# psychopa4/PFNL

Measured on AMD Instinct MI355X. Metric: HR frames/sec at 4xSR, 7-frame 128x128->512x512, higher is better.
Workload: dtype f32

## Files before the change

### include/pfnl_hip.h

```cpp
#ifndef PFNL_HIP_H
#define PFNL_HIP_H

#include <stddef.h>
#include <stdint.h>

#ifdef __cplusplus
extern "C" {
#endif

typedef struct pfnl_handle pfnl_handle;

typedef enum pfnl_status {
    PFNL_OK = 0,
    PFNL_ERR_INVALID = -1,
    PFNL_ERR_STATE = -2,
    PFNL_ERR_HIP = -3,
    PFNL_ERR_NOMEM = -4,
    PFNL_ERR_NODEVICE = -5,
    PFNL_ERR_COMM = -6,
    PFNL_ERR_RANGE = -7
} pfnl_status;

typedef struct pfnl_config {
    int32_t num_frames;
// ... 8 lines not shown
int pfnl_version(void);
int pfnl_device_count(int* count);

int pfnl_create(const pfnl_config* cfg, pfnl_handle** out);
int pfnl_destroy(pfnl_handle* h);

int pfnl_set_weight(pfnl_handle* h, const char* tf_name, const float* host,
                    const int64_t* shape, int rank);
int pfnl_missing_weights(pfnl_handle* h, int* count);
int pfnl_finalize_weights(pfnl_handle* h);

int pfnl_set_option(pfnl_handle* h, const char* key, const char* value);
int pfnl_get_option(pfnl_handle* h, const char* key, char* buf, size_t buflen);

int pfnl_forward(pfnl_handle* h, const void* in, int in_is_device, void* out, int out_is_device,
                 int B, int H, int W, void* stream);
int pfnl_forward_strip(pfnl_handle* h, const void* in, void* out, int B, int H, int W, int row0, int nrows, void* stream);
int pfnl_workspace_bytes(pfnl_handle* h, int B, int H, int W, size_t* bytes);
int pfnl_plan(pfnl_handle* h, int B, int H, int W, char* buf, size_t buflen);
int pfnl_sync(pfnl_handle* h);
int pfnl_range_reruns(pfnl_handle* h, long long* count);
int pfnl_range_flag(pfnl_handle* h, int* flagged);

int pfnl_host_alloc(size_t bytes, void** out);
int pfnl_host_free(void* p);

typedef struct pfnl_comm pfnl_comm;
#define PFNL_COMM_ID_BYTES 128
enum { PFNL_COMM_SUM = 0, PFNL_COMM_MAX = 1 };
int pfnl_comm_get_unique_id(void* id );
int pfnl_comm_init_rank(int nranks, int rank, const void* id, int device_id, pfnl_comm** out);
int pfnl_comm_init_all(int ndev, const int* devs, pfnl_comm** comms );
int pfnl_comm_destroy(pfnl_comm* c);
int pfnl_comm_rank(pfnl_comm* c, int* rank, int* nranks);
int pfnl_comm_bcast_weights(pfnl_comm* c, pfnl_handle* h, int root);
int pfnl_copy_weights(pfnl_handle* dst, pfnl_handle* src);
int pfnl_comm_bcast(pfnl_comm* c, void* dev_buf, size_t bytes, int root);
int pfnl_comm_allreduce_f64(pfnl_comm* c, double* vals, int n, int op);
int pfnl_comm_barrier(pfnl_comm* c);
int pfnl_comm_allgather(pfnl_comm* c, const float* send_dev, float* recv_dev, size_t count_per_rank, void* stream);

enum {
    PFNL_K_NL_PACK = 0, PFNL_K_NL_ATTN = 1, PFNL_K_CONV0 = 2, PFNL_K_CONV3X3 = 3,
    PFNL_K_CONV1X1 = 4, PFNL_K_MERGE1 = 5, PFNL_K_TAIL = 6, PFNL_K_COUNT = 7
};
int pfnl_profile_enable(pfnl_handle* h, int enable);
int pfnl_profile_reset(pfnl_handle* h);
int pfnl_profile_read(pfnl_handle* h, double* ms , int64_t* launches );

int pfnl_debug_tap(pfnl_handle* h, const char* name, float* host_dst, size_t count);

int pfnl_op_conv2d(const float* in, const float* kernel_host, const float* bias_host,
                   const float* addend, int add_div, const float* resid, float* out,
                   int items, int frames_per_item, int H, int W, int ksize, int cout, int act,
                   void* stream);
int pfnl_op_conv2_grouped(const float* in, const float* base, const float* kernel_host, const float* bias_host,
                          const float* resid, float* out, int clips, int frames_per_clip, int H, int W, int act,
                          void* stream);
int pfnl_op_conv3x3_accum(const float* in, const float* kernel_host, const float* bias_host, float* out, int clips,
                          int frames_per_clip, int H, int W, int cout, int act, void* stream);
int pfnl_op_conv3x3_accum_split16(const float* in, const float* kernel_host, const float* bias_host, float* out, int clips,
                                  int frames_per_clip, int H, int W, int cout, int act, void* stream);
int pfnl_op_conv1x1_stream(const float* in, const float* kernel_host, const float* bias_host, float* out,
                           int items, int frames_per_item, int HW, int act, void* stream);
int pfnl_op_conv1x1_split16(const float* in, const float* kernel_host, const float* bias_host, float* out,
                            int items, int frames_per_item, int HW, int act, void* stream);
int pfnl_op_conv3x3_bf16(const uint16_t* in, const float* kernel_host, const float* bias_host, const uint16_t* addend,
                         int add_div, const uint16_t* resid, uint16_t* out, int items, int H, int W, int act, void* stream);
int pfnl_op_conv3x3_split16(const float* in, const float* kernel_host, const float* bias_host, const float* addend, int add_div,
                            const float* resid, float* out, int items, int H, int W, int act, void* stream);
int pfnl_op_conv1_conv10_split16(const float* in, const float* k1_host, const float* b1_host, const float* k10_host,
                                 const float* b10_host, float* out1, float* base, int clips, int frames_per_clip, int H, int W,
                                 void* stream);
int pfnl_op_conv1_conv10_split16_sf0(const float* in, const float* k1_host, const float* b1_host, const float* k10_host,
                                     const float* b10_host, float* out1, float* base, int clips, int frames_per_clip, int H, int W,
                                     void* stream);
int pfnl_op_conv2_chain_sf0(const float* in, const float* kernel_host, const float* bias_host, const float* base, int add_div, const float* resid,
                            float* out, uint16_t* out_sf, int items, int H, int W, int act, void* stream);
int pfnl_op_conv2_chain_ex(const float* in, const float* kernel_host, const float* bias_host, const float* base, int add_div, const float* resid,
                           float* out, int items, int H, int W, int act, int mfma, int n_full, int split_s, int split_q, void* stream);
int pfnl_op_conv1_conv10_split16_ex(const float* in, const float* k1_host, const float* b1_host, const float* k10_host,
                                    const float* b10_host, float* out1, float* base, int clips, int frames_per_clip, int H, int W,
                                    int n_full, int split_s, int split_q, void* stream);
int pfnl_op_conv3x3_accum_split16_ex(const float* in, const float* kernel_host, const float* bias_host, float* out, int clips,
                                     int frames_per_clip, int H, int W, int cout, int act, int n_full, int split_s, int split_q, void* stream);
int pfnl_op_conv3x3_bf16_ex(const uint16_t* in, const float* kernel_host, const float* bias_host, const uint16_t* addend, int add_div,
                            const uint16_t* resid, uint16_t* out, int items, int H, int W, int act, int mfma, int n_full, int split_s,
                            int split_q, void* stream);
int pfnl_op_conv1_conv10_bf16_ex(const uint16_t* in, const float* k1_host, const float* b1_host, const float* k10_host, const float* b10_host,
                                 uint16_t* out1, uint16_t* base, int clips, int frames_per_clip, int H, int W, int mfma, int n_full, int split_s,
                                 int split_q, void* stream);
int pfnl_op_conv3x3_split16_sf(int which, const float* in, const float* kernel_host, const float* bias_host, const float* addend,
                               int add_div, const float* resid, float* out, int items, int H, int W, int act, void* stream);
int pfnl_op_conv1x1_split16_sf(const float* in, const float* kernel_host, const float* bias_host, float* out, int items,
                               int frames_per_item, int HW, int act, int in_sf, int out_sf, void* stream);
int pfnl_op_conv_small(const float* a, const float* b, int nA, int a_div, int b_mul, int nsrc, const float* kernel_host,
                       const float* bias_host, const float* resid, float* out, int items, int H, int W, int ks, int cout, int act,
                       void* stream);
int pfnl_op_conv_small_pf_block(const float* x, const float* k1_host, const float* b1_host, const float* k10_host, const float* b10_host,
                                const float* k2_host, const float* b2_host, float* inp1, float* out, int clips, int T, int H, int W,
                                void* stream);
int pfnl_op_conv1_conv10_bf16(const uint16_t* in, const float* k1_host, const float* b1_host, const float* k10_host,
                              const float* b10_host, uint16_t* out1, uint16_t* base, int clips, int frames_per_clip, int H, int W,
                              void* stream);
int pfnl_op_conv3x3_accum_bf16(const uint16_t* in, const float* kernel_host, const float* bias_host, float* out, int clips,
                               int frames_per_clip, int H, int W, int cout, int act, void* stream);
int pfnl_op_conv1x1_bf16(const uint16_t* in, const float* kernel_host, const float* bias_host, uint16_t* out, int items,
                         int frames_per_item, int HW, int act, void* stream);
int pfnl_op_conv3x3_winograd(const float* in, const float* kernel_host, const float* bias_host,
                             const float* addend, int add_div, const float* resid, float* out,
                             int items, int H, int W, int act, void* stream);
int pfnl_op_conv3x3_winograd_ws(const float* in, const float* kernel_host, const float* bias_host,
                                const float* addend, int add_div, const float* resid, float* out, int items, int H,
                                int W, int act, void* stream);
int pfnl_op_nonlocal(const float* x, const float* wg_host, const float* bg_host,
                     const float* ww_host, const float* bw_host, float* out,
                     int B, int T, int H, int W, void* stream);
int pfnl_op_nonlocal_split16(const float* x, const float* wg_host, const float* bg_host,
                     const float* ww_host, const float* bw_host, float* out,
                     int B, int T, int H, int W, void* stream);
int pfnl_op_nonlocal_f16(const float* x, const float* wg_host, const float* bg_host,
                     const float* ww_host, const float* bw_host, float* out,
                     int B, int T, int H, int W, void* stream);
int pfnl_op_nonlocal_embedded(const float* x, const float* wg_host, const float* bg_host, const float* ww_host,
                              const float* bw_host, const float* wt_host, const float* bt_host, const float* wp_host,
                              const float* bp_host, float* out, int B, int T, int H, int W, void* stream);
int pfnl_op_nonlocal_block(const float* x, const float* wg_host, const float* bg_host, const float* ww_host,
                           const float* bw_host, const float* wt_host, const float* bt_host, const float* wp_host,
                           const float* bp_host, int nltype, int sub_sample, float* out, int B, int T, int H, int W, void* stream);
int pfnl_op_conv0(const float* x, const float* kernel_host, const float* bias_host, float* out, int B, int T, int H, int W,
                  void* stream);
int pfnl_op_tail(const float* merge, const float* x, const float* kernel_host, const float* bias_host, float* out, int B,
                 int T, int H, int W, int scale, void* stream);
int pfnl_op_gather_windows(const float* frames, float* win, int F, int first, int count, int T, int H, int W, void* stream);
int pfnl_op_quantise_u8(const float* sr, uint8_t* out, size_t n, void* stream);
int pfnl_op_bicubic(const float* x, float* out, int B, int H, int W, int scale, void* stream);
int pfnl_op_blur_decimate(const float* hr, float* lr, int F, int H, int W, int scale, void* stream);
int pfnl_selftest_mfma(int device_id);

#ifdef __cplusplus
}
#endif
#endif
```

### pfnl_amd/_capi.py

```python
from __future__ import annotations

import ctypes as C
import os
from typing import Optional

_HERE = os.path.dirname(os.path.abspath(__file__))
LIB_PATH = os.environ.get("PFNL_HIP_LIB", os.path.join(_HERE, "lib", "libpfnl_hip.so"))

K_NAMES = ("nl_pack", "nl_attn", "conv0", "conv3x3", "conv1x1", "merge1", "tail")


class PFNLHipError(RuntimeError):
    """A libpfnl_hip call returned a negative status."""


class PFNLHipMissing(ImportError):
    """libpfnl_hip.so has not been built (run `python -c "import __graft_entry__ as g; g.build()"`)."""


class pfnl_config(C.Structure):
    _fields_ = [("num_frames", C.c_int32), ("scale", C.c_int32), ("mf", C.c_int32),
                ("num_block", C.c_int32), ("device_id", C.c_int32), ("reserved", C.c_int32 * 3)]


_vp, _i, _fp = C.c_void_p, C.c_int, C.POINTER(C.c_float)
SIGNATURES = {
    "pfnl_last_error": (C.c_char_p, []),
    "pfnl_version": (_i, []),
    "pfnl_device_count": (_i, [C.POINTER(_i)]),
    "pfnl_create": (_i, [C.POINTER(pfnl_config), C.POINTER(_vp)]),
    "pfnl_destroy": (_i, [_vp]),
    "pfnl_set_weight": (_i, [_vp, C.c_char_p, _vp, C.POINTER(C.c_int64), _i]),
    "pfnl_missing_weights": (_i, [_vp, C.POINTER(_i)]),
    "pfnl_finalize_weights": (_i, [_vp]),
    "pfnl_set_option": (_i, [_vp, C.c_char_p, C.c_char_p]),
    "pfnl_forward": (_i, [_vp, _vp, _i, _vp, _i, _i, _i, _i, _vp]),
    "pfnl_forward_strip": (_i, [_vp, _vp, _vp, _i, _i, _i, _i, _i, _vp]),
    "pfnl_workspace_bytes": (_i, [_vp, _i, _i, _i, C.POINTER(C.c_size_t)]),
    "pfnl_plan": (_i, [_vp, _i, _i, _i, C.c_char_p, C.c_size_t]),
    "pfnl_get_option": (_i, [_vp, C.c_char_p, C.c_char_p, C.c_size_t]),
    "pfnl_sync": (_i, [_vp]),
    "pfnl_range_reruns": (_i, [_vp, C.POINTER(C.c_longlong)]),
    "pfnl_range_flag": (_i, [_vp, C.POINTER(_i)]),
    "pfnl_host_alloc": (_i, [C.c_size_t, C.POINTER(_vp)]),
    "pfnl_host_free": (_i, [_vp]),
    "pfnl_profile_enable": (_i, [_vp, _i]),
    "pfnl_profile_reset": (_i, [_vp]),
    "pfnl_profile_read": (_i, [_vp, C.POINTER(C.c_double), C.POINTER(C.c_int64)]),
    "pfnl_debug_tap": (_i, [_vp, C.c_char_p, _vp, C.c_size_t]),
    "pfnl_op_conv2d": (_i, [_vp, _vp, _vp, _vp, _i, _vp, _vp, _i, _i, _i, _i, _i, _i, _i, _vp]),
    "pfnl_op_conv2_grouped": (_i, [_vp, _vp, _vp, _vp, _vp, _vp, _i, _i, _i, _i, _i, _vp]),
    "pfnl_op_conv3x3_accum": (_i, [_vp, _vp, _vp, _vp, _i, _i, _i, _i, _i, _i, _vp]),
    "pfnl_op_conv3x3_accum_split16": (_i, [_vp, _vp, _vp, _vp, _i, _i, _i, _i, _i, _i, _vp]),
    "pfnl_op_conv1x1_split16": (_i, [_vp, _vp, _vp, _vp, _i, _i, _i, _i, _vp]),
    "pfnl_op_conv1x1_stream": (_i, [_vp, _vp, _vp, _vp, _i, _i, _i, _i, _vp]),
    "pfnl_op_conv3x3_bf16": (_i, [_vp, _vp, _vp, _vp, _i, _vp, _vp, _i, _i, _i, _i, _vp]),
    "pfnl_op_conv1x1_bf16": (_i, [_vp, _vp, _vp, _vp, _i, _i, _i, _i, _vp]),
    "pfnl_op_conv3x3_accum_bf16": (_i, [_vp, _vp, _vp, _vp, _i, _i, _i, _i, _i, _i, _vp]),
    "pfnl_op_conv1_conv10_bf16": (_i, [_vp, _vp, _vp, _vp, _vp, _vp, _vp, _i, _i, _i, _i, _vp]),
    "pfnl_op_conv3x3_winograd": (_i, [_vp, _vp, _vp, _vp, _i, _vp, _vp, _i, _i, _i, _i, _vp]),
    "pfnl_op_conv3x3_split16": (_i, [_vp, _vp, _vp, _vp, _i, _vp, _vp, _i, _i, _i, _i, _vp]),
    "pfnl_op_conv3x3_split16_sf": (_i, [_i, _vp, _vp, _vp, _vp, _i, _vp, _vp, _i, _i, _i, _i, _vp]),
    "pfnl_op_conv_small": (_i, [_vp, _vp, _i, _i, _i, _i, _vp, _vp, _vp, _vp, _i, _i, _i, _i, _i, _i, _vp]),
    "pfnl_op_conv_small_pf_block": (_i, [_vp, _vp, _vp, _vp, _vp, _vp, _vp, _vp, _vp, _i, _i, _i, _i, _vp]),
    "pfnl_op_conv1x1_split16_sf": (_i, [_vp, _vp, _vp, _vp, _i, _i, _i, _i, _i, _i, _vp]),
    "pfnl_op_conv3x3_winograd_ws": (_i, [_vp, _vp, _vp, _vp, _i, _vp, _vp, _i, _i, _i, _i, _vp]),
    "pfnl_op_nonlocal": (_i, [_vp, _vp, _vp, _vp, _vp, _vp, _i, _i, _i, _i, _vp]),
    "pfnl_op_nonlocal_split16": (_i, [_vp, _vp, _vp, _vp, _vp, _vp, _i, _i, _i, _i, _vp]),
    "pfnl_op_nonlocal_f16": (_i, [_vp, _vp, _vp, _vp, _vp, _vp, _i, _i, _i, _i, _vp]),
    "pfnl_op_bicubic": (_i, [_vp, _vp, _i, _i, _i, _i, _vp]),
    "pfnl_op_blur_decimate": (_i, [_vp, _vp, _i, _i, _i, _i, _vp]),
    "pfnl_selftest_mfma": (_i, [_i]),
    "pfnl_op_nonlocal_embedded": (_i, [_vp, _vp, _vp, _vp, _vp, _vp, _vp, _vp, _vp, _vp, _i, _i, _i, _i, _vp]),
    "pfnl_op_conv1_conv10_split16": (_i, [_vp, _vp, _vp, _vp, _vp, _vp, _vp, _i, _i, _i, _i, _vp]),
    "pfnl_op_conv1_conv10_split16_sf0": (_i, [_vp, _vp, _vp, _vp, _vp, _vp, _vp, _i, _i, _i, _i, _vp]),
    "pfnl_op_conv2_chain_sf0": (_i, [_vp, _vp, _vp, _vp, _i, _vp, _vp, _vp, _i, _i, _i, _i, _vp]),
    "pfnl_op_conv2_chain_ex": (_i, [_vp, _vp, _vp, _vp, _i, _vp, _vp, _i, _i, _i, _i, _i, _i, _i, _i, _vp]),
    "pfnl_op_conv1_conv10_split16_ex": (_i, [_vp, _vp, _vp, _vp, _vp, _vp, _vp, _i, _i, _i, _i, _i, _i, _i, _vp]),
    "pfnl_op_conv3x3_accum_split16_ex": (_i, [_vp, _vp, _vp, _vp, _i, _i, _i, _i, _i, _i, _i, _i, _i, _vp]),
    "pfnl_op_conv3x3_bf16_ex": (_i, [_vp, _vp, _vp, _vp, _i, _vp, _vp, _i, _i, _i, _i, _i, _i, _i, _i, _vp]),
    "pfnl_op_conv1_conv10_bf16_ex": (_i, [_vp, _vp, _vp, _vp, _vp, _vp, _vp, _i, _i, _i, _i, _i, _i, _i, _i, _vp]),
    "pfnl_op_nonlocal_block": (_i, [_vp, _vp, _vp, _vp, _vp, _vp, _vp, _vp, _vp, _i, _i, _vp, _i, _i, _i, _i, _vp]),
    "pfnl_op_conv0": (_i, [_vp, _vp, _vp, _vp, _i, _i, _i, _i, _vp]),
    "pfnl_op_tail": (_i, [_vp, _vp, _vp, _vp, _vp, _i, _i, _i, _i, _i, _vp]),
    "pfnl_op_gather_windows": (_i, [_vp, _vp, _i, _i, _i, _i, _i, _i, _vp]),
    "pfnl_op_quantise_u8": (_i, [_vp, _vp, C.c_size_t, _vp]),
    "pfnl_comm_get_unique_id": (_i, [_vp]),
    "pfnl_comm_init_rank": (_i, [_i, _i, _vp, _i, C.POINTER(_vp)]),
    "pfnl_comm_init_all": (_i, [_i, C.POINTER(_i), C.POINTER(_vp)]),
    "pfnl_comm_destroy": (_i, [_vp]),
    "pfnl_comm_rank": (_i, [_vp, C.POINTER(_i), C.POINTER(_i)]),
    "pfnl_comm_bcast_weights": (_i, [_vp, _vp, _i]),
    "pfnl_copy_weights": (_i, [_vp, _vp]),
    "pfnl_comm_bcast": (_i, [_vp, _vp, C.c_size_t, _i]),
    "pfnl_comm_allreduce_f64": (_i, [_vp, C.POINTER(C.c_double), _i, _i]),
    "pfnl_comm_barrier": (_i, [_vp]),
    "pfnl_comm_allgather": (_i, [_vp, _vp, _vp, C.c_size_t, _vp]),
}
COMM_ID_BYTES = 128
COMM_SUM, COMM_MAX = 0, 1

_lib: Optional[C.CDLL] = None


def load_library(path: str = LIB_PATH) -> C.CDLL:
    global _lib
    if _lib is not None:
        return _lib
    if not os.path.exists(path):
        raise PFNLHipMissing(f"{path} not found: build it with __graft_entry__.build() "
                             f"(make -C pfnl_amd/csrc); there is no CPU fallback")
    try:
        import torch
        cand = os.path.join(os.path.dirname(torch.__file__), "lib", "librccl.so")
        if os.path.exists(cand):
            os.environ.setdefault("PFNL_RCCL_LIB", cand)
    except Exception:
        pass
    lib = C.CDLL(path, mode=C.RTLD_GLOBAL)
    for name, (res, args) in SIGNATURES.items():
        fn = getattr(lib, name)
        fn.restype = res
        fn.argtypes = args
    _lib = lib
    return lib


def check(status: int) -> None:
    if status != 0:
        msg = load_library().pfnl_last_error()
        raise PFNLHipError(f"libpfnl_hip status {status}: {msg.decode() if msg else '?'}")


def device_count() -> int:
    n = C.c_int(0)
    check(load_library().pfnl_device_count(C.byref(n)))
    return n.value
```

### pfnl_amd/csrc/capi.hip

```cpp
#include <dlfcn.h>

#include <atomic>
#include <cmath>
#include <condition_variable>
#include <cstdio>
#include <cstdlib>
#include <cstring>
#include <functional>
#include <map>
#include <memory>
#include <mutex>
#include <string>
#include <thread>
#include <vector>

#include "../../include/pfnl_hip.h"
#include "capi_internal.h"
#include "common.h"
#include "conv_bf16.h"
#include "conv_split16.h"
#include "conv_small.h"

namespace {

// ... 51 lines not shown
    }
    void release() {
        if (p) hipHostFree(p);
        p = nullptr;
        n = 0;
    }
};

struct HostPool {
    std::vector<std::thread> th;
    std::mutex m;
    std::condition_variable cv_work, cv_done;
    std::function<void(int)> fn;
    std::unique_ptr<std::atomic<int>[]> flag;
    int cap = 0, n = 0, next = 0, finished = 0, device = 0;
    bool stop = false;
    void start(int k, int dev) {
        if (!th.empty()) return;
        device = dev;
        for (int i = 0; i < k; ++i) th.emplace_back([this] { loop(); });
    }
    void loop() {
        hipSetDevice(device);
        for (;;) {
            int i;
            {
                std::unique_lock<std::mutex> lk(m);
                cv_work.wait(lk, [&] { return stop || next < n; });
                if (stop) return;
                i = next++;
            }
            fn(i);
            flag[i].store(1, std::memory_order_release);
            {
                std::lock_guard<std::mutex> lk(m);
                ++finished;
            }
            cv_done.notify_all();
        }
    }
    void run(int count, std::function<void(int)> f) {
        std::lock_guard<std::mutex> lk(m);
        if (count > cap) {
            flag.reset(new std::atomic<int>[count]);
            cap = count;
        }
        for (int i = 0; i < count; ++i) flag[i].store(0, std::memory_order_relaxed);
        fn = std::move(f);
        n = count;
        next = 0;
        finished = 0;
        cv_work.notify_all();
    }
    void wait_chunk(int i) {
        while (!flag[i].load(std::memory_order_acquire)) std::this_thread::yield();
    }
    void wait() {
        std::unique_lock<std::mutex> lk(m);
        cv_done.wait(lk, [&] { return finished >= n; });
    }
    void shutdown() {
        {
            std::lock_guard<std::mutex> lk(m);
            stop = true;
        }
        cv_work.notify_all();
        for (auto& t : th) t.join();
        th.clear();
    }
};

}

static constexpr int kSmallTiles256 = 200;
static constexpr int kMidChains256 = 136;
static int scaled_by_cus(int v256, int ncu) {
    return ncu > 0 && ncu != 256 ? std::max(1, (int)((long long)v256 * ncu / 256)) : v256;
}

struct BlockPacks {
    size_t c1_w = 0, c1_b = 0, c10_w = 0, c10_b = 0, c10_s = 0, c2a_w = 0, c2b_w = 0, c2_b = 0;
    size_t c1_u = 0, c2a_u = 0, c2b_u = 0;
    size_t bf_c1 = 0, bf_c10 = 0, bf_c2a = 0, bf_c2b = 0, bf_c1_m16 = 0, bf_c2b_m16 = 0;
    size_t s_c1 = 0, s_c2a = 0, s_c2b = 0, s_c10 = 0, s_c10f = 0, s_c2a_sf = 0, s_c2b_sf = 0, s_c2a_m16 = 0, s_c2b_m16 = 0;
    size_t sm_c1 = 0, sm_c10 = 0, sm_c2 = 0;
};

struct pfnl_handle {
    pfnl_config cfg;
    int ncu = 0;
    hipStream_t stream = nullptr;
    std::map<std::string, std::vector<int64_t>> expected;
    std::map<std::string, HostTensor> host;
    bool finalized = false;
    bool weights_external = false;
    size_t wdev_used = 0, wdev16_used = 0, wdev16s_used = 0;
    struct GraphEntry {
        int B, H, W, seen;
        hipGraph_t graph;
        hipGraphExec_t exec;
        unsigned long long alloc_gen, cfg_gen;
        unsigned long long seen_cfg_gen;
        int slot;
    };
    std::vector<GraphEntry> graphs;
    unsigned long long cfg_gen = 0;
    hipEvent_t gev = nullptr;
    int graph_mode = 0;
    bool conv2_grouped = true;
    int merge_cstride = 48;
    int conv1x1_algo = 2;
    bool bf16_fuse10 = true;
    bool bf16_m16 = true;
    bool bf16 = false;
    DevBuf wdev16;
    size_t off16_m1 = 0;
    size_t off16s_m1 = 0;
    int m1_algo = 0;
    int conv_algo = 5;
    int nl_algo = 2;
    DevBuf wdev16s;
    bool s16_m16 = true;
    size_t off16m_m1 = 0;
    unsigned* rflag_host = nullptr;
    unsigned* rflag_dev = nullptr;
    PinBuf pin_in, pin_out;
    HostPool pool;
    std::vector<hipEvent_t> d2h_ev;
    bool strict = false, strict_once = false, weights_f16_ok = true;
    long long range_reruns = 0;
    int small_mode = 0;
    bool small_c10 = true;
    DevBuf p10;
    bool sf_chain = true;
    bool sf_c10 = true;
    bool sf_mid = true;
    int sf_mid_chains = 0;
    bool sf0 = false;
    DevBuf inp0sf;
    bool split_chains = true;
    DevBuf c10part;
    bool sf_path = true;

    DevBuf wdev;
    size_t off_conv0_w = 0, off_conv0_b = 0;
    std::vector<BlockPacks> blocks;
    std::vector<size_t> off_m1_u;
    size_t off_m1_w = 0, off_m1_b = 0, off_m2_w = 0, off_m2_b = 0, off_nl_w = 0, off_nl_b = 0, off_zero = 0;

    std::map<std::string, std::vector<int64_t>> optional;
    bool nl_theta = false;
    size_t off_nl_m = 0, off_nl_c = 0;
    DevBuf Q;
    DevBuf Xs;
    int nl_type = -1;
    int nl_sub = 1;

    DevBuf nl16;
    DevBuf X, Xo, nlp, inp0, inp1, base, pb, merge, stage_in, stage_out, scratch;
    int lastB = 0, lastH = 0, lastW = 0;

    bool prof = false;
    int prof_mode = 0;
    bool prof_gate = true;
    bool chain_open = false;
    std::vector<hipEvent_t> evs;
    std::vector<int> ev_cls;
// ... 68 lines not shown
        if (h && h->prof && h->prof_gate && !h->chain_open) {
            prof_mark(h, s, -1);
            h->chain_open = true;
        }
    }
    ~ProfScope() {
        if (h && h->prof && h->prof_mode == 4) {
            h->run_cls = cls;
            ++h->run_n;
        } else if (h && h->prof && h->prof_gate) {
            prof_mark(h, s, cls);
        }
        if (ranged) roctx()->pop();
    }
};

int prof_collect(pfnl_handle* h) {
    for (size_t i = 0; i < h->evs_used; ++i) {
        const int cls = h->ev_cls[i];
        if (cls < 0 || i == 0) continue;
        if (hipEventSynchronize(h->evs[i]) != hipSuccess) return -1;
        float ms = 0.f;
        if (hipEventElapsedTime(&ms, h->evs[i - 1], h->evs[i]) != hipSuccess) return -1;
        h->prof_ms[cls] += ms;
        h->prof_n[cls] += h->ev_cnt[i];
    }
    h->evs_used = 0;
    h->chain_open = false;
    return 0;
}

int check_geometry(const pfnl_config& c) {
    if (c.num_frames != 3 && c.num_frames != 5 && c.num_frames != 7)
        return fail(PFNL_ERR_INVALID, "num_frames must be 3, 5 or 7");
    if (c.scale != 2 && c.scale != 4) return fail(PFNL_ERR_INVALID, "scale must be 2 or 4");
    if (c.mf != 64) return fail(PFNL_ERR_INVALID, "mf must be 64");
    if (c.num_block < 0 || c.num_block > 1024) return fail(PFNL_ERR_INVALID, "bad num_block");
    for (int r : c.reserved)
        if (r != 0) return fail(PFNL_ERR_INVALID, "reserved config fields must be 0");
    return 0;
}

void add_expected(pfnl_handle* h, const std::string& layer, int k, int cin, int cout) {
    h->expected["nlvsr/" + layer + "/kernel"] = {k, k, cin, cout};
    h->expected["nlvsr/" + layer + "/bias"] = {cout};
}

size_t numel(const std::vector<int64_t>& s) {
    size_t n = 1;
    for (auto d : s) n *= (size_t)d;
    return n;
}

enum Merge1Kind {
    M1_SMALL,
    M1_BF16,
    M1_SPLIT16,
    M1_SPLIT16_CUT,
    M1_WINOGRAD,
    M1_DIRECT,
};
const char* const kMerge1Names[] = {"small", "bf16", "split16", "split16_cut", "winograd", "direct"};

struct TrunkPlan {
    bool bf16 = false;
    bool strict = false;
    int nltype = 1;
    int nl_family = 0;
    bool nl_fused_pack = false;
    bool bmid = false, fuse10 = false;
    int algo = 0, conv1x1_algo = 0;
    bool sf = false;
    bool small = false, small_c10 = false;
    bool mid = false;
    bool c10_fused = false;
    bool chain = false;
    bool sf0 = false;
    bool conv2_grouped = false;
    int n_full = 0, split_s = 0, split_q = 0;
    int c1x1_launches = 0;
    int launches_per_block = 0;
    int tiles8x32 = 0, chains = 0;
    int mfma = 32;
    int merge1 = M1_DIRECT;
    int merge_stride = 48;
    size_t p10_floats = 0, inp0sf_floats = 0, c10part_floats = 0;
    const char* name = "";
};

void plan_bf16_trunk(const pfnl_handle* h, TrunkPlan& pl, int T, int grid, int mid_chains, bool fits32) {
    pl.bmid = h->sf_mid && h->bf16_fuse10 && pl.chains < mid_chains;
    pl.fuse10 = h->bf16_fuse10 && !pl.bmid;
    pl.launches_per_block = pl.fuse10 ? 3 : 4;
    pl.c1x1_launches = pl.fuse10 ? 0 : 1;
    if (pl.fuse10 && h->split_chains && fits32 && split_rule(pl.chains, T, grid, pl.n_full, pl.split_s, pl.split_q)) {
        pl.launches_per_block += 1;
        pl.c1x1_launches = 1;
    }
    pl.name = pl.bmid ? "bf16_mid4" : (pl.fuse10 ? (pl.split_s ? "bf16_3_split" : "bf16_3") : "bf16_4");
    pl.mfma = h->bf16_m16 ? 16 : 32;
    pl.merge1 = M1_BF16;
    pl.merge_stride = 64;
}

void plan_fp32_trunk(const pfnl_handle* h, TrunkPlan& pl, int B, int H, int W, int T, int grid, int mid_chains, bool fits32) {
    const int small_tiles = scaled_by_cus(kSmallTiles256, h->ncu);
    const int algo0 = h->conv_algo == 5 ? ((pl.tiles8x32 >= small_tiles && fits32) ? 4 : 3) : h->conv_algo;
    pl.algo = (pl.strict && algo0 == 4) ? 3 : algo0;
    pl.conv1x1_algo = (pl.strict && h->conv1x1_algo == 2) ? 1 : h->conv1x1_algo;
    pl.sf = pl.algo == 4 && pl.conv1x1_algo == 2 && h->sf_path;
    pl.small = !pl.strict && fits32 &&
               (h->small_mode == 1 || (h->small_mode == 0 && h->conv_algo == 5 && h->conv1x1_algo == 2 && pl.tiles8x32 < small_tiles));
    pl.small_c10 = pl.small && h->small_c10;
    if (pl.small) {
        pl.launches_per_block = pl.small_c10 ? 2 : 3;
        pl.c1x1_launches = pl.small_c10 ? 0 : 1;
        pl.name = pl.small_c10 ? "small2" : "small3";
        pl.merge1 = M1_SMALL;
        pl.merge_stride = 64;
        return;
    }
    pl.mid = pl.sf && h->sf_mid && h->conv_algo == 5 && h->sf_c10 && h->sf_chain && pl.chains < mid_chains;
    pl.c10_fused = pl.sf && h->sf_c10 && !pl.mid;
    pl.chain = pl.sf && h->sf_chain && !pl.mid;
    pl.sf0 = pl.c10_fused && pl.chain && h->sf0;
    const int wino_groups = B * ((W + 31) / 32) * ((H + 3) / 4);
    pl.conv2_grouped = pl.algo == 3 && h->conv2_grouped && wino_groups >= 224 && fits32;
    pl.launches_per_block = (pl.c10_fused ? 1 : 2) + ((pl.chain || pl.conv2_grouped) ? 1 : 2);
    pl.c1x1_launches = pl.c10_fused ? 0 : 1;
    if (pl.c10_fused && pl.chain && h->split_chains && split_rule(pl.chains, T, grid, pl.n_full, pl.split_s, pl.split_q)) {
        pl.launches_per_block += 1;
        pl.c1x1_launches = 1;
    }
    pl.mfma = (h->s16_m16 && pl.c10_fused && pl.chain && !pl.sf0 && !pl.split_s && pl.chains >= grid) ? 16 : 32;
    pl.name = pl.mid ? "mid4" : (pl.c10_fused && pl.chain) ? (pl.sf0 ? "chain2_sf0" : (pl.split_s ? "chain2_split" : "chain2"))
            : pl.algo == 4 ? (pl.launches_per_block == 3 ? "split16_3" : "split16_4")
            : pl.algo == 3 ? (pl.conv2_grouped ? "winograd_ws3" : "winograd_ws4")
            : pl.algo == 1 ? "winograd_tile4" : "direct4";
    if (pl.algo == 4 && h->m1_algo != 2 && fits32) pl.merge1 = pl.split_s ? M1_SPLIT16_CUT : M1_SPLIT16;
    else if ((pl.algo == 3 || pl.algo == 4) && wino_groups >= 224 && fits32) pl.merge1 = M1_WINOGRAD;
    pl.merge_stride = pl.merge1 == M1_DIRECT ? 48 : 64;
}

TrunkPlan trunk_plan(const pfnl_handle* h, int B, int H, int W, int Hfull) {
    TrunkPlan pl;
    const int T = h->cfg.num_frames;
    pl.bf16 = h->bf16;
    pl.strict = !h->bf16 && (h->strict || h->strict_once || !h->weights_f16_ok);
    pl.tiles8x32 = B * T * ((W + 31) / 32) * ((H + 7) / 8);
    pl.chains = pl.tiles8x32 / T;
    const int grid = persistent_grid(h->ncu);
    const int mid_chains = h->sf_mid_chains > 0 ? h->sf_mid_chains : scaled_by_cus(kMidChains256, h->ncu);
    const bool fits32 = (long long)H * W * 256 < 0x7fffffffLL;
    if (h->bf16) plan_bf16_trunk(h, pl, T, grid, mid_chains, fits32);
    else plan_fp32_trunk(h, pl, B, H, W, T, grid, mid_chains, fits32);

    const int N = (Hfull / 2) * (W / 2);
    pl.nltype = h->nl_type < 0 ? (h->nl_theta ? 0 : 1) : h->nl_type;
    pl.nl_family = (pl.nltype != 1 || h->nl_sub > 1) ? 0
                 : h->bf16 ? 2
                 : (!pl.strict && (h->nl_algo == 1 || (h->nl_algo == 2 && N >= 1024))) ? 1 : 3;
    pl.nl_fused_pack = (pl.nl_family == 1 || pl.nl_family == 2) && nl_f16_fits_one_launch(B, N);

    const size_t frame_floats = (size_t)B * T * H * W * 64;
    pl.p10_floats = pl.small_c10 ? frame_floats : 0;
    pl.inp0sf_floats = pl.sf0 ? frame_floats : 0;
    pl.c10part_floats = pl.split_s ? (size_t)(pl.chains - pl.n_full) * pl.split_s * 8 * 32 * 64 : 0;
    return pl;
}

struct Fwd {
    pfnl_handle* h;
    const TrunkPlan& pl;
    hipStream_t s;
    int B, T, F, H, W;
    const float* wd;
    const uint16_t* w16;
    const uint16_t* w16s;
};

template <class P>
void set_split_chains(P& q, const TrunkPlan& pl, float* partial) {
    q.n_full = pl.n_full;
    q.split_s = pl.split_s;
    q.split_q = pl.split_q;
    q.partial = pl.split_s ? partial : nullptr;
}

template <class P>
P split_finalize_params(const Fwd& f) {
    P q{};
    q.H = f.H;
    q.W = f.W;
    q.items = f.F;
    q.add_div = f.T;
    set_split_chains(q, f.pl, f.h->c10part.p);
    return q;
}

ConvParams direct_params(const Fwd& f, const float* in, const float* wpack, const float* bias, float* out, int cout, int frames, int act) {
    ConvParams p{};
    p.in = in;
    p.wpack = wpack;
    p.bias = bias;
    p.out = out;
    p.H = f.H;
    p.W = f.W;
    p.in_cstride = 64;
    p.out_cstride = cout;
    p.cout = cout;
    p.chunks_per_frame = 64 / CONV_CK;
    p.frames_per_item = frames;
    p.nchunks = frames * p.chunks_per_frame;
    p.add_div = 1;
    p.act = act;
    return p;
}
// ... 77 lines not shown
            q.x_bias = wd + k.c10_b;
            q.x_out = ab;
            set_split_chains(q, pl, h->c10part.p);
        }
        if (pl.mfma == 16) q.wpack16 = f.w16 + k.bf_c1_m16;
        HIPCHK(launch_conv3x3_bf16(q, s));
    }
    if (pl.fuse10 && pl.split_s) {
        ProfScope ps(h, s, PFNL_K_CONV1X1);
        ConvBf16Params q = split_finalize_params<ConvBf16Params>(f);
        q.x_bias = wd + k.c10_b;
        q.x_out = ab;
        HIPCHK(launch_c10_finalize_bf16(q, s));
    }
    if (!pl.fuse10) {
        ProfScope ps(h, s, PFNL_K_CONV1X1);
        HIPCHK(launch_conv1x1_bf16(a1, f.w16 + k.bf_c10, wd + k.c10_b, ab, f.B, f.T, f.H * f.W, 1, s));
    }
    {
        ProfScope ps(h, s, PFNL_K_CONV3X3);
        ConvBf16Params q{ab, f.w16 + k.bf_c2a, wd + h->off_zero, nullptr, nullptr, ap, f.H, f.W, f.B, 1, 0};
        HIPCHK(launch_conv3x3_bf16(q, s));
    }
    {
        ProfScope ps(h, s, PFNL_K_CONV3X3);
        ConvBf16Params q{a1, f.w16 + k.bf_c2b, wd + k.c2_b, ap, a0, a0, f.H, f.W, f.F, f.T, 1};
        q.flat = pl.bmid ? 1 : 0;
        set_split_chains(q, pl, nullptr);
        if (pl.mfma == 16) q.wpack16 = f.w16 + k.bf_c2b_m16;
        HIPCHK(launch_conv3x3_bf16(q, s));
    }
    return 0;
}

int block_small(const Fwd& f, const BlockPacks& k) {
    pfnl_handle* const h = f.h;
    const hipStream_t s = f.s;
    const float* const wd = f.wd;
    const int H = f.H, W = f.W, F = f.F, T = f.T;
    {
        ProfScope ps(h, s, PFNL_K_CONV3X3);
        ConvSmallParams q{nullptr, h->inp0.p, 0, 1, 1, 1, f.w16s + k.sm_c1, wd + k.c1_b, nullptr, h->inp1.p, H, W, F, 1, 3};
        if (f.pl.small_c10) {
            q.x_wpack = f.w16s + k.sm_c10;
            q.x_out = h->p10.p;
            q.x_T = T;
        }
        HIPCHK(launch_conv_small(q, s));
    }
    if (!f.pl.small_c10) {
        ProfScope ps(h, s, PFNL_K_CONV1X1);
        ConvSmallParams q{nullptr, h->inp1.p, 0, 1, T, T, f.w16s + k.sm_c10, wd + k.c10_b, nullptr, h->base.p, H, W, f.B, 1, 1};
        HIPCHK(launch_conv_small(q, s));
    }
    {
        ProfScope ps(h, s, PFNL_K_CONV3X3);
        ConvSmallParams q{f.pl.small_c10 ? h->p10.p : h->base.p, h->inp1.p, 1, T, 1, 2, f.w16s + k.sm_c2, wd + k.c2_b, h->inp0.p, h->inp0.p, H, W, F, 1, 3};
        if (f.pl.small_c10) {
            q.a_nsum = T;
            q.a_bias = wd + k.c10_b;
        }
        HIPCHK(launch_conv_small(q, s));
    }
    return 0;
}

int block_fp32(const Fwd& f, const BlockPacks& k, bool first, bool last) {
    pfnl_handle* const h = f.h;
    const TrunkPlan& pl = f.pl;
    const hipStream_t s = f.s;
    const float* const wd = f.wd;
    const int H = f.H, W = f.W, F = f.F, T = f.T, B = f.B, algo = pl.algo;
    const bool sf = pl.sf;
    const bool in_sf0 = pl.sf0 && !first, out_sf0 = pl.sf0 && !last;
    if (pl.c10_fused) {
        {
            ProfScope ps(h, s, PFNL_K_CONV3X3);
            ConvSplitParams q{in_sf0 ? h->inp0sf.p : h->inp0.p, f.w16s + k.s_c1, wd + k.c1_b, nullptr, nullptr, h->inp1.p, H, W, F, T, 1};
            q.in_sf = in_sf0 ? 1 : 0;
            q.wpack2 = f.w16s + k.s_c10f;
            q.bias2 = wd + k.c10_b;
            q.out2 = h->base.p;
            set_split_chains(q, pl, h->c10part.p);
            HIPCHK(launch_conv3x3_c1c10(q, s));
        }
        if (pl.split_s) {
            ProfScope ps(h, s, PFNL_K_CONV1X1);
            ConvSplitParams q = split_finalize_params<ConvSplitParams>(f);
            q.act = 1;
            q.out2 = h->base.p;
            HIPCHK(launch_c10_finalize(q, s));
        }
    } else {
        {
            ProfScope ps(h, s, PFNL_K_CONV3X3);
            if (algo == 4) {
                ConvSplitParams q{h->inp0.p, f.w16s + k.s_c1, wd + k.c1_b, nullptr, nullptr, h->inp1.p, H, W, F, 1, 1};
                q.out_sf = sf ? 1 : 0;
                HIPCHK(launch_conv3x3_split16(q, s));
            } else if (algo == 1 || algo == 3) {
                WinoParams wp{h->inp0.p, wd + k.c1_u, wd + k.c1_b, nullptr, nullptr, h->inp1.p, H, W, 1, 1, F};
                HIPCHK(algo == 3 ? launch_conv_wino_ws(wp, s) : launch_conv_wino(wp, s));
            } else {
                HIPCHK(launch_conv_mfma(direct_params(f, h->inp0.p, wd + k.c1_w, wd + k.c1_b, h->inp1.p, 64, 1, 1), 3, F, s));
            }
        }
        {
            ProfScope ps(h, s, PFNL_K_CONV1X1);
            if (pl.conv1x1_algo == 2)
                HIPCHK(launch_conv1x1_split16(h->inp1.p, f.w16s + k.s_c10, wd + k.c10_b, h->base.p, B, T, H * W, 1, s, sf, sf));
            else if (pl.conv1x1_algo == 1)
                HIPCHK(launch_conv1x1_stream(h->inp1.p, wd + k.c10_s, wd + k.c10_b, h->base.p, B, T, H * W, 1, s));
            else
                HIPCHK(launch_conv_mfma(direct_params(f, h->inp1.p, wd + k.c10_w, wd + k.c10_b, h->base.p, 64, T, 1), 1, B, s));
        }
    }
    if (pl.conv2_grouped) {
        ProfScope ps(h, s, PFNL_K_CONV3X3);
        WinoParams wp{h->inp1.p, wd + k.c2b_u, wd + k.c2_b, nullptr, h->inp0.p, h->inp0.p, H, W, T, 1, F};
        wp.in2 = h->base.p;
        wp.upack2 = wd + k.c2a_u;
        HIPCHK(launch_conv_wino_ws(wp, s));
        return 0;
    }
    if (pl.chain) {
        ProfScope ps(h, s, PFNL_K_CONV3X3);
        ConvSplitParams q{h->inp1.p, f.w16s + k.s_c2b_sf, wd + k.c2_b, nullptr, h->inp0.p, h->inp0.p, H, W, F, T, 1};
        q.in2 = h->base.p;
        q.wpack2 = f.w16s + k.s_c2a_sf;
        q.out2 = out_sf0 ? h->inp0sf.p : nullptr;
        set_split_chains(q, pl, nullptr);
        if (pl.mfma == 16) {
            q.wpack_m16 = f.w16s + k.s_c2b_m16;
            q.wpack2_m16 = f.w16s + k.s_c2a_m16;
        }
        HIPCHK(launch_conv3x3_sf_chain(q, s));
        return 0;
    }
    {
        ProfScope ps(h, s, PFNL_K_CONV3X3);
        if (algo == 4) {
            ConvSplitParams q{h->base.p, f.w16s + (sf ? k.s_c2a_sf : k.s_c2a), wd + h->off_zero, nullptr, nullptr, h->pb.p, H, W, B, 1, 0};
            HIPCHK(sf ? launch_conv3x3_sf(q, s) : launch_conv3x3_split16(q, s));
        } else if (algo == 1 || algo == 3) {
            WinoParams wp{h->base.p, wd + k.c2a_u, wd + h->off_zero, nullptr, nullptr, h->pb.p, H, W, 1, 0, B};
            HIPCHK(algo == 3 ? launch_conv_wino_ws(wp, s) : launch_conv_wino(wp, s));
        } else {
            HIPCHK(launch_conv_mfma(direct_params(f, h->base.p, wd + k.c2a_w, wd + h->off_zero, h->pb.p, 64, 1, 0), 3, B, s));
        }
    }
    {
        ProfScope ps(h, s, PFNL_K_CONV3X3);
        if (algo == 4) {
            ConvSplitParams q{h->inp1.p, f.w16s + (sf ? k.s_c2b_sf : k.s_c2b), wd + k.c2_b, h->pb.p, h->inp0.p, h->inp0.p, H, W, F, T, 1};
            q.flat = pl.mid ? 1 : 0;
            HIPCHK(sf ? launch_conv3x3_sf(q, s) : launch_conv3x3_split16(q, s));
        } else if (algo == 1 || algo == 3) {
            WinoParams wp{h->inp1.p, wd + k.c2b_u, wd + k.c2_b, h->pb.p, h->inp0.p, h->inp0.p, H, W, T, 1, F};
            HIPCHK(algo == 3 ? launch_conv_wino_ws(wp, s) : launch_conv_wino(wp, s));
        } else {
            ConvParams p = direct_params(f, h->inp1.p, wd + k.c2b_w, wd + k.c2_b, h->inp0.p, 64, 1, 1);
            p.addend = h->pb.p;
            p.add_div = T;
            p.resid = h->inp0.p;
            HIPCHK(launch_conv_mfma(p, 3, F, s));
        }
// ... 392 lines not shown
    h->blocks.assign(nb, BlockPacks{});
    for (int i = 0; i < nb; ++i) {
        const std::string s = std::to_string(i);
        BlockPacks& k = h->blocks[i];
        k.c1_w = put_pack(W("conv1_" + s), 3, 64, 0, 64, 64);
        k.c1_b = put_bias(Bv("conv1_" + s));
        k.c10_w = put_pack(W("conv10_" + s), 1, 64 * T, 0, 64 * T, 64);
        k.c10_b = put_bias(Bv("conv10_" + s));
        k.c10_s = reserve(pfnl::conv1x1_pack_floats(T));
        pfnl::conv1x1_pack_weights(W("conv10_" + s).data(), T, &blob[k.c10_s]);
        k.c2a_w = put_pack(W("conv2_" + s), 3, 128, 0, 64, 64);
        k.c2b_w = put_pack(W("conv2_" + s), 3, 128, 64, 64, 64);
        k.c2_b = put_bias(Bv("conv2_" + s));
        k.c1_u = put_wino(W("conv1_" + s), 64, 0);
        k.c2a_u = put_wino(W("conv2_" + s), 128, 0);
        k.c2b_u = put_wino(W("conv2_" + s), 128, 64);
    }
    h->off_m1_w = put_pack(W("convmerge1"), 3, 64 * T, 0, 64 * T, 48);
    h->off_m1_b = put_bias(Bv("convmerge1"));
    h->off_m1_u.assign(T, 0);
    for (int f = 0; f < T; ++f) {
        h->off_m1_u[f] = reserve(pfnl::wino_pack_floats());
        pfnl::wino_pack_weights(W("convmerge1").data(), 64 * T, 64 * f, &blob[h->off_m1_u[f]], 48);
    }
    {
        const auto& k = W("convmerge2");
        h->off_m2_w = reserve(k.size());
        std::memcpy(&blob[h->off_m2_w], k.data(), k.size() * sizeof(float));
        h->off_m2_b = put_bias(Bv("convmerge2"));
    }
    {
        h->off_nl_w = reserve((size_t)CP * CP);
        h->off_nl_b = reserve(CP);
        pfnl_nl_fold_gw(W("nlblock_0/g/g").data(), Bv("nlblock_0/g/g").data(), W("nlblock_0/w/w").data(), Bv("nlblock_0/w/w").data(), C, CP,
                        &blob[h->off_nl_w], &blob[h->off_nl_b]);
    }
    {
        int have = 0;
        for (auto& kv : h->optional) have += (int)h->host.count(kv.first);
        if (have != 0 && have != (int)h->optional.size())
            return fail(PFNL_ERR_STATE, "nlblock_0 theta/phi: all four tensors (two kernels, two biases) or none");
        h->nl_theta = have != 0;
        if (h->nl_theta) {
            h->off_nl_m = reserve((size_t)CP * CP);
            h->off_nl_c = reserve(CP);
            pfnl_nl_fold_theta_phi(W("nlblock_0/theta/theta").data(), Bv("nlblock_0/theta/theta").data(), W("nlblock_0/phi/phi").data(),
                                   Bv("nlblock_0/phi/phi").data(), C, CP, &blob[h->off_nl_m], &blob[h->off_nl_c]);
        }
    }
    {
        std::vector<uint16_t> b16;
        auto reserve16 = [&](size_t n) {
            size_t off = (b16.size() + 127) / 128 * 128;
            b16.resize(off + n, 0);
            return off;
        };
        for (int i = 0; i < nb; ++i) {
            const std::string s = std::to_string(i);
            BlockPacks& k = h->blocks[i];
            k.bf_c1 = reserve16(pfnl::conv3x3_bf16_pack_halfs());
            pfnl::conv3x3_bf16_pack_weights(W("conv1_" + s).data(), 64, 0, &b16[k.bf_c1]);
            k.bf_c10 = reserve16(pfnl::conv1x1_bf16_pack_halfs(T));
            pfnl::conv1x1_bf16_pack_weights(W("conv10_" + s).data(), T, &b16[k.bf_c10]);
            k.bf_c2a = reserve16(pfnl::conv3x3_bf16_pack_halfs());
            pfnl::conv3x3_bf16_pack_weights(W("conv2_" + s).data(), 128, 0, &b16[k.bf_c2a]);
            k.bf_c2b = reserve16(pfnl::conv3x3_bf16_pack_halfs());
            pfnl::conv3x3_bf16_pack_weights(W("conv2_" + s).data(), 128, 64, &b16[k.bf_c2b]);
            k.bf_c1_m16 = reserve16(pfnl::conv3x3_bf16_pack_halfs());
            pfnl::conv3x3_bf16_pack_weights16(W("conv1_" + s).data(), 64, 0, &b16[k.bf_c1_m16]);
            k.bf_c2b_m16 = reserve16(pfnl::conv3x3_bf16_pack_halfs());
            pfnl::conv3x3_bf16_pack_weights16(W("conv2_" + s).data(), 128, 64, &b16[k.bf_c2b_m16]);
        }
        h->off16_m1 = reserve16((size_t)T * pfnl::conv3x3_bf16_pack_halfs());
        for (int f = 0; f < T; ++f)
            pfnl::conv3x3_bf16_pack_weights(W("convmerge1").data(), 64 * T, 64 * f, &b16[h->off16_m1 + (size_t)f * pfnl::conv3x3_bf16_pack_halfs()], 48);
        b16.resize((b16.size() + 1) / 2 * 2 + 2, 0);
        h->wdev16_used = b16.size() / 2;
        if (h->wdev16.ensure(b16.size() / 2)) return fail(PFNL_ERR_NOMEM, "weight allocation failed");
        HIPCHK(hipMemcpy(h->wdev16.p, b16.data(), b16.size() * sizeof(uint16_t), hipMemcpyHostToDevice));
    }
    {
        std::vector<uint16_t> b16;
        const size_t n3 = pfnl::conv3x3_split16_pack_halfs(), n1 = pfnl::conv1x1_split16_pack_halfs(T);
        const size_t blk = 7 * n3 + n1 + pfnl::conv1x1_c10_pack_halfs(T);
        h->off16s_m1 = (size_t)nb * blk;
        const size_t m3 = pfnl::conv_small_pack_halfs(3, 1), m10 = pfnl::conv_small_pack_halfs(1, T);
        const size_t small_base = (size_t)nb * blk + (size_t)T * n3;
        h->off16m_m1 = small_base + (size_t)nb * (3 * m3 + m10);
        b16.resize(h->off16m_m1 + (size_t)T * m3 + 2, 0);
        pfnl::conv_small_pack_weights(W("convmerge1").data(), 3, T, 48, &b16[h->off16m_m1]);
        for (int f = 0; f < T; ++f)
            pfnl::conv3x3_split16_pack_weights(W("convmerge1").data(), 64 * T, 64 * f, &b16[h->off16s_m1 + (size_t)f * n3], 48);
        for (int i = 0; i < nb; ++i) {
            const std::string s = std::to_string(i);
            BlockPacks& k = h->blocks[i];
            k.s_c1 = (size_t)i * blk;
            k.s_c2a = k.s_c1 + n3;
            k.s_c2b = k.s_c1 + 2 * n3;
            k.s_c10 = k.s_c1 + 3 * n3;
            k.s_c2a_sf = k.s_c10 + n1;
            k.s_c2b_sf = k.s_c2a_sf + n3;
            k.s_c10f = k.s_c2b_sf + n3;
            k.s_c2a_m16 = k.s_c10f + pfnl::conv1x1_c10_pack_halfs(T);
            k.s_c2b_m16 = k.s_c2a_m16 + n3;
            pfnl::conv3x3_split16_pack_weights16(W("conv2_" + s).data(), 128, 0, &b16[k.s_c2a_m16]);
            pfnl::conv3x3_split16_pack_weights16(W("conv2_" + s).data(), 128, 64, &b16[k.s_c2b_m16]);
            pfnl::conv1x1_c10_pack_weights(W("conv10_" + s).data(), T, &b16[k.s_c10f]);
            pfnl::conv3x3_split16_pack_weights(W("conv2_" + s).data(), 128, 0, &b16[k.s_c2a_sf], 64, true);
            pfnl::conv3x3_split16_pack_weights(W("conv2_" + s).data(), 128, 64, &b16[k.s_c2b_sf], 64, true);
            k.sm_c1 = small_base + (size_t)i * (3 * m3 + m10);
            k.sm_c2 = k.sm_c1 + m3;
            k.sm_c10 = k.sm_c1 + 3 * m3;
            pfnl::conv_small_pack_weights(W("conv1_" + s).data(), 3, 1, 64, &b16[k.sm_c1]);
            pfnl::conv_small_pack_weights(W("conv2_" + s).data(), 3, 2, 64, &b16[k.sm_c2]);
            pfnl::conv_small_pack_weights(W("conv10_" + s).data(), 1, T, 64, &b16[k.sm_c10]);
            pfnl::conv1x1_split16_pack_weights(W("conv10_" + s).data(), T, &b16[k.s_c10]);
            pfnl::conv3x3_split16_pack_weights(W("conv1_" + s).data(), 64, 0, &b16[k.s_c1]);
            pfnl::conv3x3_split16_pack_weights(W("conv2_" + s).data(), 128, 0, &b16[k.s_c2a]);
            pfnl::conv3x3_split16_pack_weights(W("conv2_" + s).data(), 128, 64, &b16[k.s_c2b]);
        }
        h->wdev16s_used = b16.size() / 2;
        if (h->wdev16s.ensure(b16.size() / 2)) return fail(PFNL_ERR_NOMEM, "weight allocation failed");
        HIPCHK(hipMemcpy(h->wdev16s.p, b16.data(), b16.size() / 2 * 2 * sizeof(uint16_t), hipMemcpyHostToDevice));
    }
    {
        float wmax = 0.f;
        for (const auto& kv : h->host)
            for (float v : kv.second.data) wmax = std::fmax(wmax, std::fabs(v));
        h->weights_f16_ok = wmax < 65504.0f;
    }
    h->wdev_used = blob.size();
    if (h->wdev.ensure(blob.size())) return fail(PFNL_ERR_NOMEM, "weight allocation failed");
    HIPCHK(hipMemcpy(h->wdev.p, blob.data(), blob.size() * sizeof(float), hipMemcpyHostToDevice));
    h->finalized = true;
    ++h->cfg_gen;
    return 0;
}

int pfnl_workspace_bytes(pfnl_handle* h, int B, int H, int W, size_t* bytes) {
    if (!h || !bytes) return fail(PFNL_ERR_INVALID, "NULL argument");
    if (B <= 0 || H <= 0 || W <= 0 || (H & 1) || (W & 1)) return fail(PFNL_ERR_INVALID, "bad shape");
    const size_t T = h->cfg.num_frames, P = (size_t)H * W, N = P / 4, sc = h->cfg.scale;
    const int C = 12 * (int)T;
    const size_t CP = pfnl::nl_padded_ch(C);
    size_t f = 2 * B * N * CP
             + pfnl::nl_partial_floats(B, (int)N, C)
             + 2 * B * T * P * 64
             + 3 * B * P * 64
             + (size_t)B * T * P * 3 + (size_t)B * P * sc * sc * 3;
    if (h->bf16 || h->nl_algo != 0) f += (pfnl::nl_f16_scratch_halfs(B, (int)N) + 1) / 2;
    if (h->nl_theta) f += (size_t)B * N * CP;
    if (h->nl_sub > 1) f += (size_t)B * ((H / 2) / h->nl_sub) * ((W / 2) / h->nl_sub) * CP;
    const TrunkPlan pl = trunk_plan(h, B, H, W, H);
    f += pl.p10_floats + pl.inp0sf_floats + pl.c10part_floats;
    *bytes = f * sizeof(float);
    return 0;
}

int pfnl_plan(pfnl_handle* h, int B, int H, int W, char* buf, size_t buflen) {
    if (!h || !buf || buflen < 1) return fail(PFNL_ERR_INVALID, "NULL argument");
    if (B <= 0 || H <= 0 || W <= 0 || (H & 1) || (W & 1)) return fail(PFNL_ERR_INVALID, "bad shape");
    const TrunkPlan pl = trunk_plan(h, B, H, W, H);
    static const char* const nln[] = {"general_f32", "split16", "f16", "f32"};
    static const char* const a3[] = {"direct", "winograd_tile", "?", "winograd", "split16"};
    static const char* const a1[] = {"tiled", "stream", "split16"};
    char tmp[384];
    if (pl.bf16)
        std::snprintf(tmp, sizeof tmp, "%s launches_per_block=%d c1x1=%d precision=bf16 tiles=%d chains=%d whole_chains=%d split_parts=%d part_frames=%d nl=%s nl_pack_fused=%d mfma=%d merge1=%s",
                      pl.name, pl.launches_per_block, pl.c1x1_launches, pl.tiles8x32, pl.chains, pl.split_s ? pl.n_full : pl.chains, pl.split_s, pl.split_q,
                      nln[pl.nl_family], pl.nl_fused_pack ? 1 : 0, pl.mfma, kMerge1Names[pl.merge1]);
    else
        std::snprintf(tmp, sizeof tmp, "%s launches_per_block=%d c1x1=%d precision=fp32 conv3x3=%s conv1x1=%s c10_fused=%d chain=%d sf0=%d strict=%d tiles=%d chains=%d "
                      "whole_chains=%d split_parts=%d part_frames=%d nl=%s nl_pack_fused=%d mfma=%d merge1=%s",
                      pl.name, pl.launches_per_block, pl.c1x1_launches, pl.small ? "small" : a3[pl.algo < 0 || pl.algo > 4 ? 2 : pl.algo],
                      a1[pl.conv1x1_algo < 0 || pl.conv1x1_algo > 2 ? 0 : pl.conv1x1_algo], pl.c10_fused ? 1 : 0, pl.chain ? 1 : 0, pl.sf0 ? 1 : 0,
                      pl.strict ? 1 : 0, pl.tiles8x32, pl.chains, pl.split_s ? pl.n_full : pl.chains, pl.split_s, pl.split_q, nln[pl.nl_family],
                      pl.nl_fused_pack ? 1 : 0, pl.mfma, kMerge1Names[pl.merge1]);
    if (std::strlen(tmp) + 1 > buflen) return fail(PFNL_ERR_INVALID, "buffer too small");
    std::strcpy(buf, tmp);
    return 0;
}

static int range_flag_take(pfnl_handle* h, int slot, int* flagged) {
    unsigned* const f = h->rflag_host + slot;
    *flagged = __atomic_exchange_n(f, 0u, __ATOMIC_ACQ_REL) != 0;
    return 0;
}

int pfnl_range_reruns(pfnl_handle* h, long long* count) {
    if (!h || !count) return fail(PFNL_ERR_INVALID, "NULL argument");
    *count = h->range_reruns;
    return 0;
}

namespace {
constexpr size_t STAGE_POOL_MIN = 512u << 10;
constexpr int STAGE_MAX_CHUNKS = 32;

bool host_is_pinned(const void* p) {
    hipPointerAttribute_t a;
    if (hipPointerGetAttributes(&a, p) != hipSuccess) {
        (void)hipGetLastError();
        return false;
    }
    return a.type == hipMemoryTypeHost;
}

void ensure_pool(pfnl_handle* h) {
    if (!h->pool.th.empty()) return;
    int k = 4;
    if (const char* e = std::getenv("PFNL_HOST_THREADS")) k = std::atoi(e);
    const int hw = (int)std::thread::hardware_concurrency();
    if (hw > 1 && k > hw - 1) k = hw - 1;
    k = k < 1 ? 1 : (k > 16 ? 16 : k);
    h->pool.start(k, h->cfg.device_id);
}

size_t stage_chunk_bytes(size_t bytes) {
    size_t c = (bytes + STAGE_MAX_CHUNKS - 1) / STAGE_MAX_CHUNKS;
    if (c < (1u << 20)) c = 1u << 20;
    return (c + 4095) & ~(size_t)4095;
}

int stage_h2d(pfnl_handle* h, float* dst, const void* src, size_t bytes, hipStream_t s) {
    if (host_is_pinned(src)) {
        HIPCHK(hipMemcpyAsync(dst, src, bytes, hipMemcpyHostToDevice, s));
        return 0;
    }
    if (h->pin_in.ensure(bytes)) return fail(PFNL_ERR_NOMEM, "pinned staging allocation failed");
    unsigned char* const pin = h->pin_in.p;
    if (bytes < STAGE_POOL_MIN) {
        std::memcpy(pin, src, bytes);
        HIPCHK(hipMemcpyAsync(dst, pin, bytes, hipMemcpyHostToDevice, s));
        return 0;
    }
    ensure_pool(h);
    const size_t csz = stage_chunk_bytes(bytes);
    const int n = (int)((bytes + csz - 1) / csz);
    const unsigned char* const sp = static_cast<const unsigned char*>(src);
    h->pool.run(n, [=](int i) {
        const size_t off = (size_t)i * csz;
        std::memcpy(pin + off, sp + off, std::min(csz, bytes - off));
    });
    hipError_t err = hipSuccess;
    for (int i = 0; i < n; ++i) {
        h->pool.wait_chunk(i);
        const size_t off = (size_t)i * csz;
        if (err == hipSuccess)
            err = hipMemcpyAsync(reinterpret_cast<unsigned char*>(dst) + off, pin + off, std::min(csz, bytes - off), hipMemcpyHostToDevice, s);
    }
    h->pool.wait();
    if (err != hipSuccess) return fail(PFNL_ERR_HIP, std::string("H2D staging: ") + hipGetErrorString(err));
    return 0;
}

int stage_d2h(pfnl_handle* h, void* dst, const float* src, size_t bytes, hipStream_t s) {
    if (host_is_pinned(dst)) {
        HIPCHK(hipMemcpyAsync(dst, src, bytes, hipMemcpyDeviceToHost, s));
        HIPCHK(hipStreamSynchronize(s));
        return 0;
// ... 367 lines not shown
```

### pfnl_amd/csrc/capi_ops.hip

```cpp
#include <cstring>
#include <string>
#include <vector>

#include "../../include/pfnl_hip.h"
#include "capi_internal.h"
#include "common.h"
#include "conv_bf16.h"
#include "conv_small.h"
#include "conv_split16.h"

namespace {

int fail(int code, const std::string& msg) { return pfnl_internal_fail(code, msg); }

class OpStage {
  public:
    explicit OpStage(void* stream) : s(static_cast<hipStream_t>(stream)) {}
    OpStage(const OpStage&) = delete;
    OpStage& operator=(const OpStage&) = delete;
    ~OpStage() {
        for (void* p : bufs) (void)hipFree(p);
    }

    const hipStream_t s;
// ... 46 lines not shown
}
static size_t split_partial_floats(int H, int W, int items, int T, int n_full, int split_s) {
    const size_t nchains = (size_t)((W + 31) / 32) * ((H + 7) / 8) * (items / T);
    return (nchains - (size_t)n_full) * split_s * 8 * 32 * 64;
}

static int op_conv3x3_accum_split16(const float* in, const float* kernel_host, const float* bias_host, float* out, int clips,
                                    int frames_per_clip, int H, int W, int cout, int act, void* stream, int n_full = 0, int split_s = 0,
                                    int split_q = 0) {
    OpStage st(stream);
    const int T = frames_per_clip;
    const size_t nh = pfnl::conv3x3_split16_pack_halfs();
    std::vector<uint16_t> pack((size_t)T * nh + 128, 0);
    for (int f = 0; f < T; ++f) pfnl::conv3x3_split16_pack_weights(kernel_host, 64 * T, 64 * f, pack.data() + (size_t)f * nh, cout);
    if (bias_host) std::memcpy(&pack[(size_t)T * nh], bias_host, cout * sizeof(float));
    uint16_t* dw = st.upload(pack);
    float* part = split_s ? st.alloc<float>(split_partial_floats(H, W, clips * T, T, n_full, split_s)) : nullptr;
    st.run([&] {
        pfnl::ConvSplitParams q{in, dw, reinterpret_cast<const float*>(dw + (size_t)T * nh), nullptr, nullptr, out, H, W, clips * T, T, act, 1};
        q.n_full = n_full;
        q.split_s = split_s;
        q.split_q = split_q;
        q.partial = part;
        return pfnl::launch_conv3x3_split16(q, st.s);
    });
    if (split_s) st.run([&] {
        pfnl::ConvSplitParams f{};
        f.H = H;
        f.W = W;
        f.items = clips * T;
        f.add_div = T;
        f.act = act;
        f.n_full = n_full;
        f.split_s = split_s;
        f.split_q = split_q;
        f.partial = part;
        f.bias = reinterpret_cast<const float*>(dw + (size_t)T * nh);
        f.out = out;
        return pfnl::launch_c10_finalize(f, st.s);
    });
    return st.finish("accumulating conv (split16) op: ");
}

static int op_conv2_chain(const float* in, const float* kernel_host, const float* bias_host, const float* addend, int add_div, const float* resid,
                          float* out, uint16_t* out_sf, int items, int H, int W, int act, void* stream,
                          int mfma = 32, int n_full = 0, int split_s = 0, int split_q = 0) {
    OpStage st(stream);
    const size_t nh2 = pfnl::conv3x3_split16_pack_halfs();
    const bool m16 = mfma == 16;
    std::vector<uint16_t> pk((m16 ? 4 : 2) * nh2 + 128, 0);
    pfnl::conv3x3_split16_pack_weights(kernel_host, 128, 0, pk.data(), 64, true);
    pfnl::conv3x3_split16_pack_weights(kernel_host, 128, 64, pk.data() + nh2, 64, true);
    if (bias_host) std::memcpy(&pk[2 * nh2], bias_host, 64 * sizeof(float));
    if (m16) {
        pfnl::conv3x3_split16_pack_weights16(kernel_host, 128, 0, pk.data() + 2 * nh2 + 128);
        pfnl::conv3x3_split16_pack_weights16(kernel_host, 128, 64, pk.data() + 3 * nh2 + 128);
    }
    const size_t npf = (size_t)items * H * W, npb = (size_t)(items / add_div) * H * W;
    uint16_t* dw2 = st.upload(pk);
    uint16_t* tf = st.alloc<uint16_t>(npf * 128);
    uint16_t* tb = st.alloc<uint16_t>(npb * 128);
    st.run([&] { return pfnl::launch_sf_from_f32(in, tf, npf, st.s); });
    st.run([&] { return pfnl::launch_sf_from_f32(addend, tb, npb, st.s); });
    if (out != resid) st.run([&] { return hipMemcpyAsync(out, resid, npf * 256, hipMemcpyDeviceToDevice, st.s); });
    st.run([&] {
        pfnl::ConvSplitParams q{reinterpret_cast<const float*>(tf), dw2 + nh2, reinterpret_cast<const float*>(dw2 + 2 * nh2), nullptr, out, out, H, W, items, add_div, act};
        q.in2 = reinterpret_cast<const float*>(tb);
        q.wpack2 = dw2;
        q.out2 = reinterpret_cast<float*>(out_sf);
        q.n_full = n_full;
        q.split_s = split_s;
        q.split_q = split_q;
        if (m16) {
            q.wpack_m16 = dw2 + 3 * nh2 + 128;
            q.wpack2_m16 = dw2 + 2 * nh2 + 128;
        }
        return pfnl::launch_conv3x3_sf_chain(q, st.s);
    });
    return st.finish("conv2 chain op: ");
}

static int op_conv1_conv10_split16(const float* in, const float* k1_host, const float* b1_host, const float* k10_host,
                                   const float* b10_host, float* out1, float* base, int clips, int frames_per_clip, int H, int W,
                                   void* stream, bool in_sf, int n_full = 0, int split_s = 0, int split_q = 0) {
    if (!in || !k1_host || !k10_host || !out1 || !base) return fail(PFNL_ERR_INVALID, "NULL argument");
    const int T = frames_per_clip;
    if (clips < 1 || T < 1 || T > 7 || H < 1 || W < 1) return fail(PFNL_ERR_INVALID, "unsupported conv geometry");
    OpStage st(stream);
    const size_t n3 = pfnl::conv3x3_split16_pack_halfs(), n1 = pfnl::conv1x1_c10_pack_halfs(T);
    std::vector<uint16_t> pack(n3 + n1 + 256, 0);
    pfnl::conv3x3_split16_pack_weights(k1_host, 64, 0, pack.data());
    pfnl::conv1x1_c10_pack_weights(k10_host, T, pack.data() + n3);
    if (b1_host) std::memcpy(&pack[n3 + n1], b1_host, 64 * sizeof(float));
    if (b10_host) std::memcpy(&pack[n3 + n1 + 128], b10_host, 64 * sizeof(float));
    const size_t np1 = (size_t)clips * T * H * W, npb = (size_t)clips * H * W;
    uint16_t* dw = st.upload(pack);
    uint16_t* t1 = st.alloc<uint16_t>(np1 * 128);
    uint16_t* tb = st.alloc<uint16_t>(npb * 128);
    uint16_t* ti = in_sf ? st.alloc<uint16_t>(np1 * 128) : nullptr;
    float* part = split_s ? st.alloc<float>(split_partial_floats(H, W, clips * T, T, n_full, split_s)) : nullptr;
    if (in_sf) st.run([&] { return pfnl::launch_sf_from_f32(in, ti, np1, st.s); });
    st.run([&] {
        pfnl::ConvSplitParams q{in_sf ? reinterpret_cast<const float*>(ti) : in, dw, reinterpret_cast<const float*>(dw + n3 + n1), nullptr, nullptr, reinterpret_cast<float*>(t1), H, W, clips * T, T, 1};
        q.in_sf = in_sf ? 1 : 0;
        q.wpack2 = dw + n3;
        q.bias2 = reinterpret_cast<const float*>(dw + n3 + n1 + 128);
        q.out2 = reinterpret_cast<float*>(tb);
        q.n_full = n_full;
        q.split_s = split_s;
        q.split_q = split_q;
        q.partial = part;
        return pfnl::launch_conv3x3_c1c10(q, st.s);
    });
    if (split_s) st.run([&] {
        pfnl::ConvSplitParams f{};
        f.H = H;
        f.W = W;
        f.items = clips * T;
        f.add_div = T;
        f.act = 1;
        f.n_full = n_full;
        f.split_s = split_s;
        f.split_q = split_q;
        f.partial = part;
        f.out2 = reinterpret_cast<float*>(tb);
        return pfnl::launch_c10_finalize(f, st.s);
    });
    st.run([&] { return pfnl::launch_sf_to_f32(t1, out1, np1, st.s); });
    st.run([&] { return pfnl::launch_sf_to_f32(tb, base, npb, st.s); });
    return st.finish("conv1+conv10 split16 op: ");
}

static int op_bf16_v3(int mode, const uint16_t* in, const float* k_host, const float* b_host, const uint16_t* addend, int add_div,
                      const uint16_t* resid, uint16_t* out, const float* k10_host, const float* b10_host, uint16_t* base, int items, int H,
                      int W, int act, int mfma, int n_full, int split_s, int split_q, void* stream) {
    OpStage st(stream);
    const int T = add_div;
    const size_t n3 = pfnl::conv3x3_bf16_pack_halfs(), n1 = mode == 2 ? pfnl::conv1x1_bf16_pack_halfs(T) : 0;
    std::vector<uint16_t> pack(2 * n3 + n1 + 256, 0);
    pfnl::conv3x3_bf16_pack_weights(k_host, 64, 0, pack.data());
    pfnl::conv3x3_bf16_pack_weights16(k_host, 64, 0, pack.data() + n3);
    if (mode == 2) pfnl::conv1x1_bf16_pack_weights(k10_host, T, pack.data() + 2 * n3);
    if (b_host) std::memcpy(&pack[2 * n3 + n1], b_host, 64 * sizeof(float));
    if (b10_host) std::memcpy(&pack[2 * n3 + n1 + 128], b10_host, 64 * sizeof(float));
    uint16_t* dw = st.upload(pack);
    float* part = mode == 2 && split_s ? st.alloc<float>(split_partial_floats(H, W, items, T, n_full, split_s)) : nullptr;
    if (!st.ok()) return st.finish("bf16 v3 op: ");
    const float* const db = reinterpret_cast<const float*>(dw + 2 * n3 + n1);
    pfnl::ConvBf16Params q{in, dw, db, addend, resid, out, H, W, items, T, act};
    if (mode == 2) {
        q.x_w = dw + 2 * n3;
        q.x_bias = db + 64;
        q.x_out = base;
    }
    q.n_full = n_full;
    q.split_s = split_s;
    q.split_q = split_q;
    q.partial = part;
    if (mfma == 16) q.wpack16 = dw + n3;
    st.run([&] { return pfnl::launch_conv3x3_bf16_v3(q, mode, st.s); });
    if (mode == 2 && split_s) st.run([&] { return pfnl::launch_c10_finalize_bf16(q, st.s); });
    return st.finish("bf16 v3 op: ");
}

static int op_conv3x3_wino(bool ws, const float* in, const float* kernel_host, const float* bias_host,
                           const float* addend, int add_div, const float* resid, float* out, int items, int H,
                           int W, int act, void* stream) {
    if (!in || !kernel_host || !out) return fail(PFNL_ERR_INVALID, "NULL argument");
    if (items < 1 || H < 2 || W < 2 || (H & 1) || (W & 1)) return fail(PFNL_ERR_INVALID, "winograd conv needs even H, W");
    if (!paired(addend, resid)) return fail(PFNL_ERR_INVALID, "addend and resid must be given together or not at all");
    if (addend && add_div < 1) return fail(PFNL_ERR_INVALID, "add_div must be >= 1");
    OpStage st(stream);
    std::vector<float> pack(pfnl::wino_pack_floats() + 64, 0.f);
    pfnl::wino_pack_weights(kernel_host, 64, 0, pack.data());
    const size_t boff = pack.size() - 64;
    if (bias_host) std::memcpy(&pack[boff], bias_host, 64 * sizeof(float));
    float* dw = st.upload(pack);
    if (!st.ok()) return st.finish("winograd conv op: ");
    pfnl::WinoParams wp{in, dw, dw + boff, addend, resid, out, H, W, addend ? add_div : 1, act, items};
    st.run([&] { return ws ? pfnl::launch_conv_wino_ws(wp, st.s) : pfnl::launch_conv_wino(wp, st.s); });
    return st.finish("winograd conv op: ");
}

static int op_nonlocal(int bf16 , const float* x, const float* wg, const float* bg, const float* ww, const float* bw,
                       float* out, int B, int T, int H, int W, void* stream) {
    if (!x || !wg || !bg || !ww || !bw || !out) return fail(PFNL_ERR_INVALID, "NULL argument");
    if ((T != 3 && T != 5 && T != 7) || B < 1 || H < 2 || W < 2 || (H & 1) || (W & 1))
        return fail(PFNL_ERR_INVALID, "unsupported non-local geometry");
    OpStage st(stream);
    const int C = 12 * T, CP = pfnl::nl_padded_ch(C), N = (H / 2) * (W / 2);
    std::vector<float> blob((size_t)CP * CP + CP, 0.f);
    pfnl_nl_fold_gw(wg, bg, ww, bw, C, CP, blob.data(), blob.data() + (size_t)CP * CP);
    const size_t nX = (size_t)B * N * CP;
    const size_t nP = pfnl::nl_partial_floats(B, N, C);
// ... 322 lines not shown
    st.run([&] {
        pfnl::ConvSmallParams q{part, inp1, 1, T, 1, 2, dw + n1 + n10, db + 128, x, out, H, W, (int)F, 1, 3};
        q.a_nsum = T;
        q.a_bias = db + 64;
        return pfnl::launch_conv_small(q, st.s);
    });
    return st.finish("conv_small block op: ");
}

int pfnl_op_conv2_chain_sf0(const float* in, const float* kernel_host, const float* bias_host, const float* base, int add_div, const float* resid,
                            float* out, uint16_t* out_sf, int items, int H, int W, int act, void* stream) {
    if (!in || !kernel_host || !out || !out_sf || !base || !resid) return fail(PFNL_ERR_INVALID, "NULL argument");
    if (items < 1 || H < 1 || W < 1 || add_div < 1 || items % add_div) return fail(PFNL_ERR_INVALID, "unsupported conv geometry");
    return op_conv2_chain(in, kernel_host, bias_host, base, add_div, resid, out, out_sf, items, H, W, act, stream);
}

int pfnl_op_conv3x3_split16_sf(int which, const float* in, const float* kernel_host, const float* bias_host, const float* addend,
                               int add_div, const float* resid, float* out, int items, int H, int W, int act, void* stream) {
    if (!in || !kernel_host || !out) return fail(PFNL_ERR_INVALID, "NULL argument");
    if (which < 0 || which > 2 || items < 1 || H < 1 || W < 1 || !paired(addend, resid)) return fail(PFNL_ERR_INVALID, "unsupported conv geometry");
    if (addend && ((which != 0 && which != 2) || add_div < 1 || items % add_div)) return fail(PFNL_ERR_INVALID, "fused mode: which = 0 or 2, items a multiple of add_div");
    if (which == 2) {
        if (!addend) return fail(PFNL_ERR_INVALID, "which = 2 needs base (addend argument) and resid");
        return op_conv2_chain(in, kernel_host, bias_host, addend, add_div, resid, out, nullptr, items, H, W, act, stream);
    }
    OpStage st(stream);
    const size_t nh = pfnl::conv3x3_split16_pack_halfs();
    std::vector<uint16_t> pack(nh + 128, 0);
    pfnl::conv3x3_split16_pack_weights(kernel_host, 64, 0, pack.data(), 64, which == 0);
    if (bias_host) std::memcpy(&pack[nh], bias_host, 64 * sizeof(float));
    const size_t npix = (size_t)items * H * W;
    uint16_t* dw = st.upload(pack);
    uint16_t* tmp = st.alloc<uint16_t>(npix * 128);
    if (which == 0) {
        st.run([&] { return pfnl::launch_sf_from_f32(in, tmp, npix, st.s); });
        st.run([&] {
            pfnl::ConvSplitParams q{reinterpret_cast<const float*>(tmp), dw, reinterpret_cast<const float*>(dw + nh), addend, resid, out, H, W, items, add_div < 1 ? 1 : add_div, act};
            return pfnl::launch_conv3x3_sf(q, st.s);
        });
    } else {
        st.run([&] {
            pfnl::ConvSplitParams q{in, dw, reinterpret_cast<const float*>(dw + nh), nullptr, nullptr, reinterpret_cast<float*>(tmp), H, W, items, 1, act};
            q.out_sf = 1;
            return pfnl::launch_conv3x3_split16(q, st.s);
        });
        st.run([&] { return pfnl::launch_sf_to_f32(tmp, out, npix, st.s); });
    }
    return st.finish("conv3x3 split16 SF op: ");
}

int pfnl_op_conv1_conv10_split16(const float* in, const float* k1_host, const float* b1_host, const float* k10_host,
                                 const float* b10_host, float* out1, float* base, int clips, int frames_per_clip, int H, int W,
                                 void* stream) {
    return op_conv1_conv10_split16(in, k1_host, b1_host, k10_host, b10_host, out1, base, clips, frames_per_clip, H, W, stream, false);
}
int pfnl_op_conv1_conv10_split16_sf0(const float* in, const float* k1_host, const float* b1_host, const float* k10_host,
                                     const float* b10_host, float* out1, float* base, int clips, int frames_per_clip, int H, int W,
                                     void* stream) {
    return op_conv1_conv10_split16(in, k1_host, b1_host, k10_host, b10_host, out1, base, clips, frames_per_clip, H, W, stream, true);
}

int pfnl_op_conv2_chain_ex(const float* in, const float* kernel_host, const float* bias_host, const float* base, int add_div, const float* resid,
                           float* out, int items, int H, int W, int act, int mfma, int n_full, int split_s, int split_q, void* stream) {
    if (!in || !kernel_host || !out || !base || !resid) return fail(PFNL_ERR_INVALID, "NULL argument");
    if (items < 1 || H < 1 || W < 1 || add_div < 1 || items % add_div) return fail(PFNL_ERR_INVALID, "unsupported conv geometry");
    if (int r = frame_too_large(H, W, 256)) return r;
    if (mfma != 16 && mfma != 32) return fail(PFNL_ERR_INVALID, "mfma must be 16 or 32");
    if (mfma == 16 && split_s) return fail(PFNL_ERR_INVALID, "split chains run on the 32x32x16 kernel only");
    if (!split_args_ok(H, W, items, add_div, n_full, split_s, split_q)) return fail(PFNL_ERR_INVALID, "invalid split-chain geometry");
    return op_conv2_chain(in, kernel_host, bias_host, base, add_div, resid, out, nullptr, items, H, W, act, stream, mfma, n_full, split_s, split_q);
}

int pfnl_op_conv1_conv10_split16_ex(const float* in, const float* k1_host, const float* b1_host, const float* k10_host,
                                    const float* b10_host, float* out1, float* base, int clips, int frames_per_clip, int H, int W,
                                    int n_full, int split_s, int split_q, void* stream) {
    if (!in || !k1_host || !k10_host || !out1 || !base) return fail(PFNL_ERR_INVALID, "NULL argument");
    const int T = frames_per_clip;
    if (clips < 1 || T < 1 || T > 7 || H < 1 || W < 1) return fail(PFNL_ERR_INVALID, "unsupported conv geometry");
    if (int r = frame_too_large(H, W, 256)) return r;
    if (!split_args_ok(H, W, clips * T, T, n_full, split_s, split_q)) return fail(PFNL_ERR_INVALID, "invalid split-chain geometry");
    return op_conv1_conv10_split16(in, k1_host, b1_host, k10_host, b10_host, out1, base, clips, T, H, W, stream, false, n_full, split_s, split_q);
}

int pfnl_op_conv3x3_accum_split16_ex(const float* in, const float* kernel_host, const float* bias_host, float* out, int clips,
                                     int frames_per_clip, int H, int W, int cout, int act, int n_full, int split_s, int split_q, void* stream) {
    if (!in || !kernel_host || !out) return fail(PFNL_ERR_INVALID, "NULL argument");
    if (clips < 1 || frames_per_clip < 1 || H < 1 || W < 1 || cout < 1 || cout > 64) return fail(PFNL_ERR_INVALID, "accumulating conv needs cout <= 64");
    if (int r = frame_too_large(H, W, 256)) return r;
    if (!split_args_ok(H, W, clips * frames_per_clip, frames_per_clip, n_full, split_s, split_q)) return fail(PFNL_ERR_INVALID, "invalid split-chain geometry");
    return op_conv3x3_accum_split16(in, kernel_host, bias_host, out, clips, frames_per_clip, H, W, cout, act, stream, n_full, split_s, split_q);
}

int pfnl_op_conv3x3_bf16_ex(const uint16_t* in, const float* kernel_host, const float* bias_host, const uint16_t* addend, int add_div,
                            const uint16_t* resid, uint16_t* out, int items, int H, int W, int act, int mfma, int n_full, int split_s,
                            int split_q, void* stream) {
    if (!in || !kernel_host || !addend || !resid || !out) return fail(PFNL_ERR_INVALID, "NULL argument");
    if (items < 1 || H < 1 || W < 1 || add_div < 1 || items % add_div) return fail(PFNL_ERR_INVALID, "unsupported conv geometry");
    if (int r = frame_too_large(H, W, 128)) return r;
    if (mfma != 16 && mfma != 32) return fail(PFNL_ERR_INVALID, "mfma must be 16 or 32");
    if (!split_args_ok(H, W, items, add_div, n_full, split_s, split_q)) return fail(PFNL_ERR_INVALID, "invalid split-chain geometry");
    return op_bf16_v3(1, in, kernel_host, bias_host, addend, add_div, resid, out, nullptr, nullptr, nullptr, items, H, W, act, mfma, n_full,
                      split_s, split_q, stream);
}

int pfnl_op_conv1_conv10_bf16_ex(const uint16_t* in, const float* k1_host, const float* b1_host, const float* k10_host, const float* b10_host,
                                 uint16_t* out1, uint16_t* base, int clips, int frames_per_clip, int H, int W, int mfma, int n_full, int split_s,
                                 int split_q, void* stream) {
    if (!in || !k1_host || !k10_host || !out1 || !base) return fail(PFNL_ERR_INVALID, "NULL argument");
    const int T = frames_per_clip;
    if (clips < 1 || (T != 3 && T != 5 && T != 7) || H < 1 || W < 1) return fail(PFNL_ERR_INVALID, "unsupported conv geometry");
    if (int r = frame_too_large(H, W, 128)) return r;
    if (mfma != 16 && mfma != 32) return fail(PFNL_ERR_INVALID, "mfma must be 16 or 32");
    if (!split_args_ok(H, W, clips * T, T, n_full, split_s, split_q)) return fail(PFNL_ERR_INVALID, "invalid split-chain geometry");
    return op_bf16_v3(2, in, k1_host, b1_host, nullptr, T, nullptr, out1, k10_host, b10_host, base, clips * T, H, W, 1, mfma, n_full, split_s,
                      split_q, stream);
}

int pfnl_op_conv1x1_split16_sf(const float* in, const float* kernel_host, const float* bias_host, float* out, int items,
                               int frames_per_item, int HW, int act, int in_sf, int out_sf, void* stream) {
    if (!in || !kernel_host || !out) return fail(PFNL_ERR_INVALID, "NULL argument");
    if (items < 1 || frames_per_item < 1 || HW < 1) return fail(PFNL_ERR_INVALID, "unsupported conv geometry");
    OpStage st(stream);
    const int T = frames_per_item;
    const size_t nh = pfnl::conv1x1_split16_pack_halfs(T);
    std::vector<uint16_t> pack(nh + 128, 0);
    pfnl::conv1x1_split16_pack_weights(kernel_host, T, pack.data());
    if (bias_host) std::memcpy(&pack[nh], bias_host, 64 * sizeof(float));
    const size_t npin = (size_t)items * T * HW, npout = (size_t)items * HW;
    uint16_t* dw = st.upload(pack);
    uint16_t* tin = st.alloc<uint16_t>(npin * 128);
    uint16_t* tout = st.alloc<uint16_t>(npout * 128);
    if (in_sf) st.run([&] { return pfnl::launch_sf_from_f32(in, tin, npin, st.s); });
    st.run([&] {
        return pfnl::launch_conv1x1_split16(in_sf ? reinterpret_cast<const float*>(tin) : in, dw, reinterpret_cast<const float*>(dw + nh),
                                            out_sf ? reinterpret_cast<float*>(tout) : out, items, T, HW, act, st.s, in_sf != 0, out_sf != 0);
    });
    if (out_sf) st.run([&] { return pfnl::launch_sf_to_f32(tout, out, npout, st.s); });
    return st.finish("conv1x1 split16 SF op: ");
}

int pfnl_op_conv1x1_stream(const float* in, const float* kernel_host, const float* bias_host, float* out, int items,
                           int frames_per_item, int HW, int act, void* stream) {
    if (!in || !kernel_host || !out) return fail(PFNL_ERR_INVALID, "NULL argument");
    if (items < 1 || frames_per_item < 1 || HW < 1) return fail(PFNL_ERR_INVALID, "unsupported conv geometry");
    OpStage st(stream);
    const int T = frames_per_item;
    std::vector<float> pack(pfnl::conv1x1_pack_floats(T) + 64, 0.f);
    pfnl::conv1x1_pack_weights(kernel_host, T, pack.data());
    const size_t boff = pack.size() - 64;
    if (bias_host) std::memcpy(&pack[boff], bias_host, 64 * sizeof(float));
    float* dw = st.upload(pack);
    st.run([&] { return pfnl::launch_conv1x1_stream(in, dw, dw + boff, out, items, T, HW, act, st.s); });
    return st.finish("conv1x1 op: ");
}

int pfnl_op_conv3x3_winograd(const float* in, const float* kernel_host, const float* bias_host,
                             const float* addend, int add_div, const float* resid, float* out, int items, int H,
                             int W, int act, void* stream) {
    return op_conv3x3_wino(false, in, kernel_host, bias_host, addend, add_div, resid, out, items, H, W, act, stream);
}

int pfnl_op_conv3x3_winograd_ws(const float* in, const float* kernel_host, const float* bias_host,
                                const float* addend, int add_div, const float* resid, float* out, int items, int H,
                                int W, int act, void* stream) {
    return op_conv3x3_wino(true, in, kernel_host, bias_host, addend, add_div, resid, out, items, H, W, act, stream);
}
// ... 100 lines not shown
```

### pfnl_amd/csrc/conv_split16.h

```cpp
#pragma once
#include <hip/hip_runtime.h>
#include <stddef.h>
#include <stdint.h>

#include "chain_order.h"

namespace pfnl {

struct ConvSplitParams {
    const float* in;
    const uint16_t* wpack;
    const float* bias;
    const float* addend;
    const float* resid;
    float* out;
    int H, W, items, add_div, act;
    int accum;
    int out_sf;
    const float* in2;
    const uint16_t* wpack2;
    const float* bias2;
    float* out2;
    int n_full, split_s, split_q;
    float* partial;
    int in_sf;
    int flat;
    const uint16_t* wpack_m16;
    const uint16_t* wpack2_m16;
};

hipError_t launch_conv3x3_split16(const ConvSplitParams& p, hipStream_t s);
size_t conv3x3_split16_pack_halfs();
void conv3x3_split16_pack_weights16(const float* hwio, int cin_total, int cin_begin, uint16_t* dst);
void conv3x3_split16_pack_weights(const float* hwio, int cin_total, int cin_begin, uint16_t* dst, int cout = 64,
                                  bool identity_rows = false);

hipError_t launch_conv3x3_c1c10(const ConvSplitParams& p, hipStream_t s);
hipError_t launch_c10_finalize(const ConvSplitParams& p, hipStream_t s);
size_t conv1x1_c10_pack_halfs(int T);
void conv1x1_c10_pack_weights(const float* hwio, int T, uint16_t* dst);

hipError_t launch_conv3x3_sf(const ConvSplitParams& p, hipStream_t s);
hipError_t launch_conv3x3_sf_chain(const ConvSplitParams& p, hipStream_t s);
hipError_t launch_sf_from_f32(const float* in, uint16_t* out, size_t npix, hipStream_t s);
hipError_t launch_sf_to_f32(const uint16_t* in, float* out, size_t npix, hipStream_t s);

size_t nl_f16_scratch_halfs(int B, int N);
hipError_t launch_nl_attn_f16(const float* X, float* Xo, const float* Wp, const float* bp, float* partial, uint16_t* scratch16,
                              int B, int N, int C, hipStream_t s, int q0 = 0, int q1 = -1, bool split = true,
                              bool prepacked = false);
bool nl_f16_fits_one_launch(int B, int N);
hipError_t launch_nl_pack_fused(const float* x, float* X, uint16_t* scratch16, int B, int T, int H, int W, hipStream_t s);

}
```

### pfnl_amd/csrc/conv_split16.hip

```cpp
#include <cstring>
#include <type_traits>
#include <vector>

#include "common.h"
#include "conv_split16.h"

namespace pfnl {

constexpr int CS_OUT_AUX = 17;
constexpr int CS_RESID_AUX = 0;
constexpr int CS_HALO_AUX = 0;
constexpr bool CS_LATE_FINISH = true;

typedef _Float16 h8 __attribute__((ext_vector_type(8)));
typedef _Float16 h4 __attribute__((ext_vector_type(4)));
typedef unsigned u32x4 __attribute__((ext_vector_type(4)));
typedef unsigned u32x2 __attribute__((ext_vector_type(2)));

constexpr int CS_THREADS = 512;
constexpr int CS_TH = CHAIN_TH, CS_TW = CHAIN_TW;
constexpr int CS_IH = CS_TH + 2, CS_IW = CS_TW + 2;
constexpr int CS_TILE_BYTES = CS_IH * CS_IW * 128;
constexpr int CS_W_BYTES = 3 * 2 * 3 * 2 * 2 * 1024;
constexpr int CS_SLOT_BYTES = CS_W_BYTES / 3;
// ... 429 lines not shown
                    }
                    ex0p = c_x0;
                    ey0p = c_y0;
                    eitemp = c_item / gT;
                }
                pending = last;
                fch = last ? ((SPLIT && kt + 1 == cs.nfull_tiles) ? cs.sp_f0 : 0) : fch + 1;
                c_item = n_item;
                c_y0 = n_y0;
                c_x0 = n_x0;
            }
            if constexpr (PAR == 1 && !ACCUM) {
#pragma unroll
                for (int n = 0; n < 2; ++n) accp[n] = accm[n] + accc[n] * CS_ISCALE;
                ex0p = c_x0;
                ey0p = c_y0;
                eitemp = c_item;
                c_item = n_item;
                c_y0 = n_y0;
                c_x0 = n_x0;
                pending = true;
            }
            CS_BARRIER();
        };
        unit(std::integral_constant<int, 0>{});
        unit(std::integral_constant<int, 1>{});
    }

    if constexpr (SPLIT) {
        if (cs.has_part) {
            float* const pt = p.partial + (size_t)cs.slot * (CS_TH * CS_TW * 64);
#pragma unroll
            for (int n = 0; n < 2; ++n) {
                unsigned char* const scratch = cs_smem + n * CS_TILE_BYTES;
                dump(scratch, n, 0);
                dump(scratch, n, 1);
                __syncthreads();
#pragma unroll
                for (int k = 0; k < 4; ++k) {
                    piece_read(scratch, k);
                    *reinterpret_cast<f32x4*>(pt + ((size_t)(2 * k + n) * CS_TW + (tid >> 4)) * 64 + (tid & 15) * 4) = pv;
                }
            }
            return;
        }
    }
#pragma unroll
    for (int n = 0; n < 2; ++n) {
        unsigned char* const scratch = cs_smem + n * CS_TILE_BYTES;
        piece_setup(n);
        fuse_request(0);
        fuse_request(1);
        dump(scratch, n, 0);
        dump(scratch, n, 1);
        __syncthreads();
        store_piece(scratch, 0);
        store_piece(scratch, 1);
        fuse_request(2);
        fuse_request(3);
        store_piece(scratch, 2);
        store_piece(scratch, 3);
    }
#undef CS_COMMIT1
#undef CS_REQ_SETUP
#undef CS_REQUEST_ALL
#undef CS_HALF
}


__device__ __forceinline__ void k1_dma16(__amdgpu_buffer_rsrc_t rs, unsigned lds_dst, int voff, int soff) {
    unsigned keep;
    asm volatile("s_mov_b32 %0, m0\n\ts_mov_b32 m0, %2\n\ts_nop 0\n\tbuffer_load_dwordx4 %1, %3, %4 offen lds\n\ts_mov_b32 m0, %0"
                 : "=&s"(keep) : "v"(voff), "s"(lds_dst), "s"(rs), "s"(soff) : "memory");
}

constexpr int K1_W10_AT = 16;
constexpr int K1_LDS_BYTES = CS_LDS_BYTES + 64 * 4;
constexpr int K1_DMA_NDMA = (CS_IH * CS_IW + 7) / 8;
constexpr int K1_DMA_ITERS = (K1_DMA_NDMA + 7) / 8;
constexpr int K1_SF_TILE_BYTES = K1_DMA_NDMA * 1024;
constexpr int K1_SF_LDS_BYTES = 2 * K1_SF_TILE_BYTES + CS_W_BYTES + 2 * 64 * 4;
static_assert(K1_SF_LDS_BYTES <= 160 * 1024, "LDS budget");

template <bool ISF, bool SPLIT>
__global__ __launch_bounds__(CS_THREADS, 1) void conv3x3_c1c10_kernel(ConvSplitParams p) {
    constexpr int TILE_BYTES = ISF ? K1_SF_TILE_BYTES : CS_TILE_BYTES;
    extern __shared__ __attribute__((aligned(16))) unsigned char cs_smem[];
    unsigned char* const wl = cs_smem + 2 * TILE_BYTES;
    float* const bl = reinterpret_cast<float*>(cs_smem + 2 * TILE_BYTES + CS_W_BYTES);
    float* const bl2 = bl + 64;
    const int tid = threadIdx.x;
    const int lane = tid & 63;
    const int wave = __builtin_amdgcn_readfirstlane(tid >> 6);
    if (wave >= 4) __builtin_amdgcn_s_setprio(1);
    const int rp = wave >> 1;
    const int mt = wave & 1;
    const int H = p.H, W = p.W;
    const int tiles_x = (W + CS_TW - 1) / CS_TW, tiles_y = (H + CS_TH - 1) / CS_TH;
    const int per_item = tiles_x * tiles_y;
    const int item_bytes = H * W * 256;
    const int gT = p.add_div;
    const int nchains = per_item * (p.items / gT);
    ChainShare<SPLIT> cs(blockIdx.x & 7, blockIdx.x >> 3, gridDim.x >> 3, nchains, p.n_full);
    if (cs.idle()) return;
    cs.deal(gT, p.split_s, p.split_q);
    const int nt = cs.nt;
    if (SPLIT && nt <= 0) return;
    auto decode = [&](int k, int& item, int& y0, int& x0, int& fr) __attribute__((always_inline)) {
        int ch;
        cs.tile(k, gT, ch, fr);
        chain_tile(ch, per_item, tiles_x, gT, fr, item, y0, x0);
    };

    u32x4 w0reg[CS_W_BYTES / 16 / CS_THREADS];
#pragma unroll
    for (int k = 0; k < CS_W_BYTES / 16 / CS_THREADS; ++k) w0reg[k] = reinterpret_cast<const u32x4*>(p.wpack)[k * CS_THREADS + tid];
    const float bias_r = tid < 64 ? p.bias[tid] : (tid < 128 ? p.bias2[tid - 64] : 0.f);

    [[maybe_unused]] int lpk[CS_ITERS];
    const int wbytes = W * 256;
    [[maybe_unused]] int dpk[K1_DMA_ITERS];
    if constexpr (ISF) {
#pragma unroll
        for (int k = 0; k < K1_DMA_ITERS; ++k) {
            const int pix = 8 * (wave + 8 * k) + (lane >> 3);
            const int py = pix / CS_IW, px = pix - py * CS_IW;
            dpk[k] = py | (px << 8);
        }
    }
    [[maybe_unused]] const unsigned lds0 = (unsigned)(uintptr_t)cs_smem;
#define K1_DMA_HALO(rs_, org_, interior_, y0_, x0_, buf_)                                        \
    do {                                                                                         \
        _Pragma("unroll") for (int k_ = 0; k_ < K1_DMA_ITERS; ++k_) {                            \
            const int i_ = wave + 8 * k_;                                                        \
            if (k_ < K1_DMA_ITERS - 1 || i_ < K1_DMA_NDMA) {                                     \
                const int py_ = dpk[k_] & 0xff, px_ = dpk[k_] >> 8;                              \
                const int gy_ = (y0_) + py_ - 1, gx_ = (x0_) + px_ - 1;                          \
                const bool in_ = (interior_) || ((unsigned)gy_ < (unsigned)H && (unsigned)gx_ < (unsigned)W && py_ < CS_IH); \
                const int rel_ = py_ * wbytes + px_ * 256 + (((lane & 7) ^ ((px_ >> 1) & 7)) << 4); \
                k1_dma16(rs_, lds0 + (buf_) * TILE_BYTES + i_ * 1024, in_ ? (org_) + rel_ : 0x7fffffff, 0); \
            }                                                                                    \
        }                                                                                        \
    } while (0)
#pragma unroll
    for (int k = 0; k < (ISF ? 0 : CS_ITERS); ++k) {
        const int id = k * CS_THREADS + tid < CS_PIECES ? k * CS_THREADS + tid : CS_PIECES - 8 + (tid & 7);
        int pix = id >> 3;
        const int c = id & 7;
        if (pix < (CS_IH * CS_IW & ~15)) pix = (pix & ~15) | ((pix & 1) << 3) | ((pix & 15) >> 1);
        const int py = pix / CS_IW, px = pix - py * CS_IW;
        lpk[k] = ((py * CS_IW + px) * 128 + 8 * (c & 1) + (((c >> 1) ^ ((px >> 1) & 7)) << 4)) | (py << 16) | (px << 24);
    }
    const int c16 = (tid & 7) * 16;
    const float nscale = __builtin_bit_cast(float, __builtin_amdgcn_readfirstlane(__builtin_bit_cast(int, -CS_SCALE)));
    [[maybe_unused]] f32x4 stg[CS_ITERS];
#define K1_REQUEST_ALL(rs_, org_, interior_, y0_, x0_)                                           \
    do {                                                                                         \
        _Pragma("unroll") for (int k_ = 0; k_ < CS_ITERS; ++k_) {                                \
            const int py_ = (lpk[k_] >> 16) & 0xff, px_ = (unsigned)lpk[k_] >> 24;               \
            const int gy_ = (y0_) + py_ - 1, gx_ = (x0_) + px_ - 1;                              \
            const bool in_ = (interior_) | (((unsigned)gy_ < (unsigned)H) & ((unsigned)gx_ < (unsigned)W));    \
            const int off_ = (org_) + py_ * wbytes + px_ * 256 + c16;                            \
            K1_HALO_LOAD(stg[k_], rs_, in_ ? off_ : 0x7fffffff);                                  \
        }                                                                                        \
    } while (0)
#define K1_HALO_LOAD(dst_, rs_, off_) do { dst_ = __builtin_bit_cast(f32x4, __builtin_amdgcn_raw_buffer_load_b128(rs_, off_, 0, CS_HALO_AUX)); } while (0)
#define K1_COMMIT1(k_, buf_)                                                                     \
    do {                                                                                         \
        u32x2 hi_, lo2_;                                                                         \
        split4(stg[k_], hi_, lo2_, nscale);                                                      \
        const int lo_ = lpk[k_] & 0xffff;                                                        \
        *reinterpret_cast<u32x2*>(cs_smem + (buf_) * TILE_BYTES + lo_) = hi_;                    \
        *reinterpret_cast<u32x2*>(cs_smem + (buf_) * TILE_BYTES + (lo_ ^ 64)) = lo2_;            \
    } while (0)

    int paddr[3];
#pragma unroll
    for (int kx = 0; kx < 3; ++kx) {
        const int col = (lane & 31) + kx;
        paddr[kx] = ((2 * rp) * CS_IW + col) * 128 + ((((lane >> 5)) ^ ((col >> 1) & 7)) << 4);
    }
    const int lo_xor = 4 << 4;
    const unsigned char* const wlane = wl + mt * 2048 + lane * 16;
    const int kh = lane >> 5;
    const int ech = 32 * mt + 16 * kh;
    f32x16 accm[2], accc[2], base_m[2];
    u32x4 held[8];
    int hx0 = 0, hy0 = 0, hitem = 0;
    bool hpend = false;
#pragma unroll
    for (int n = 0; n < 2; ++n)
#pragma unroll
        for (int r = 0; r < 16; ++r) {
            accm[n][r] = 0.f;
            accc[n][r] = 0.f;
        }
    const float slope = p.act ? 0.2f : 1.0f;

    const unsigned ldsw = (unsigned)(uintptr_t)wl;
    const int wvoff = wave * 1024 + lane * 16;
#define K1_DMA_W(half_, slot_)                                                                   \
    do {                                                                                         \
        const __amdgpu_buffer_rsrc_t rw_ = __builtin_amdgcn_make_buffer_rsrc(const_cast<uint16_t*>(p.wpack), 0, 2 * CS_W_BYTES, 0x00020000); \
        _Pragma("unroll") for (int k_ = 0; k_ < 3; ++k_)                                         \
            k1_dma16(rw_, ldsw + (slot_) * CS_SLOT_BYTES + (wave + 8 * k_) * 1024, wvoff, (half_) * CS_W_BYTES + (slot_) * CS_SLOT_BYTES + k_ * 8192); \
    } while (0)
#define K1_BARRIER() asm volatile("s_waitcnt lgkmcnt(0)\n\ts_barrier" ::: "memory")

    unsigned char* const scratch = cs_smem + TILE_BYTES;
    struct RowHalves { u32x2 hi[4], lo[4]; };
    auto quarter_prep = [&](RowHalves& h, const f32x16& m, const f32x16& c, int q, bool fold) __attribute__((always_inline)) {
        f32x4 t = {m[4 * q], m[4 * q + 1], m[4 * q + 2], m[4 * q + 3]};
        if (fold) t += f32x4{c[4 * q], c[4 * q + 1], c[4 * q + 2], c[4 * q + 3]} * CS_ISCALE;
        else asm volatile("" : "+v"(t));
        const f32x4 st = mul4s(t, slope);
        asm("v_max_f32 %0, %1, %2" : "=v"(t.x) : "v"(t.x), "v"(st.x));
        asm("v_max_f32 %0, %1, %2" : "=v"(t.y) : "v"(t.y), "v"(st.y));
        asm("v_max_f32 %0, %1, %2" : "=v"(t.z) : "v"(t.z), "v"(st.z));
        asm("v_max_f32 %0, %1, %2" : "=v"(t.w) : "v"(t.w), "v"(st.w));
        split4(t, h.hi[q], h.lo[q], nscale);
    };
    const int pp = rp * 32 + (lane & 31);
    const int sw = pp & 15;
    unsigned char* const pl = scratch + pp * 256;
    auto row_dump = [&](const RowHalves& h) __attribute__((always_inline)) {
        const int c0 = 8 * mt + 2 * kh;
        *reinterpret_cast<u32x4*>(pl + ((c0 ^ sw) << 4)) = u32x4{h.hi[0].x, h.hi[0].y, h.hi[1].x, h.hi[1].y};
        *reinterpret_cast<u32x4*>(pl + (((c0 + 1) ^ sw) << 4)) = u32x4{h.hi[2].x, h.hi[2].y, h.hi[3].x, h.hi[3].y};
        *reinterpret_cast<u32x4*>(pl + (((c0 + 4) ^ sw) << 4)) = u32x4{h.lo[0].x, h.lo[0].y, h.lo[1].x, h.lo[1].y};
        *reinterpret_cast<u32x4*>(pl + (((c0 + 5) ^ sw) << 4)) = u32x4{h.lo[2].x, h.lo[2].y, h.lo[3].x, h.lo[3].y};
    };
    auto row_pass = [&](int n, auto mm, const u32x4 (&w10)[8], u32x4* pc, auto&& fill) __attribute__((always_inline)) {
        constexpr bool MM = decltype(mm)::value;
#pragma unroll
        for (int i = 0; i < 4; ++i) {
            const int id = i * CS_THREADS + tid, ppx = id >> 4, c = id & 15;
            pc[i] = *reinterpret_cast<const u32x4*>(scratch + ppx * 256 + ((c ^ (ppx & 15)) << 4));
        }
        if constexpr (MM) {
            h8 bh[4], bo[4];
#pragma unroll
            for (int q = 0; q < 4; ++q) {
                const int cb = 8 * (q >> 1) + 2 * kh + (q & 1);
                bh[q] = *reinterpret_cast<const h8*>(pl + ((cb ^ sw) << 4));
                bo[q] = *reinterpret_cast<const h8*>(pl + (((cb + 4) ^ sw) << 4));
            }
            f32x16 cross;
#pragma unroll
            for (int r = 0; r < 16; ++r) cross[r] = 0.f;
            __builtin_amdgcn_sched_barrier(0);
#pragma unroll
            for (int q = 0; q < 4; ++q) {
                const h8 ah = __builtin_bit_cast(h8, w10[2 * q]), ao = __builtin_bit_cast(h8, w10[2 * q + 1]);
                cross = mfma_f16(ao, bh[q], cross);
                base_m[n] = mfma_f16(ah, bh[q], base_m[n]);
                cross = mfma_f16(ah, bo[q], cross);
                __builtin_amdgcn_sched_barrier(0);
                fill(q);
                __builtin_amdgcn_sched_barrier(0);
            }
            base_m[n] += cross * CS_ISCALE;
        }
    };
    auto held_store = [&](int j, float* base_ptr) __attribute__((always_inline)) {
        const __amdgpu_buffer_rsrc_t rsO = __builtin_amdgcn_make_buffer_rsrc(base_ptr + (size_t)hitem * H * W * 64, 0, item_bytes, 0x00020000);
        const int id = (j & 3) * CS_THREADS + tid, ppx = id >> 4, c = id & 15;
        const int gy = hy0 + 2 * (ppx >> 5) + (j >> 2), gx = hx0 + (ppx & 31);
        const int off = (gy * W + gx) * 256 + c * 16;
        buffer_store_b128_guarded<CS_OUT_AUX>(held[j], rsO, (hpend & (gx < W)) ? off : 0x7fffffff, 0);
    };
    auto base_init = [&](bool zero) __attribute__((always_inline)) {
#pragma unroll
        for (int n = 0; n < 2; ++n)
#pragma unroll
            for (int r = 0; r < 16; ++r) base_m[n][r] = zero ? 0.f : bl2[ech + r];
    };

    int c_item, c_y0, c_x0, n_item, n_y0, n_x0, fch, n_f;
    decode(0, c_item, c_y0, c_x0, fch);
    n_item = c_item;
    n_y0 = c_y0;
    n_x0 = c_x0;
    n_f = fch;
    {
        const __amdgpu_buffer_rsrc_t rs = __builtin_amdgcn_make_buffer_rsrc(
            const_cast<float*>(p.in) + (size_t)c_item * H * W * 64, 0, item_bytes, 0x00020000);
        const int org = ((c_y0 - 1) * W + c_x0 - 1) * 256;
        [[maybe_unused]] const bool interior = c_y0 > 0 && c_y0 + CS_IH - 1 <= H && c_x0 > 0 && c_x0 + CS_IW - 1 <= W;
        [[maybe_unused]] unsigned fence0 = 0;
        if constexpr (ISF) {
            K1_DMA_HALO(rs, org, false, c_y0, c_x0, 0);
            fence0 = __builtin_amdgcn_raw_buffer_load_b32(rs, 0, 0, 0);
        } else {
            K1_REQUEST_ALL(rs, org, interior, c_y0, c_x0);
        }
#pragma unroll
        for (int k = 0; k < CS_W_BYTES / 16 / CS_THREADS; ++k) reinterpret_cast<u32x4*>(wl)[k * CS_THREADS + tid] = w0reg[k];
        if (tid < 128) bl[tid] = bias_r;
        if constexpr (ISF) {
            asm volatile("" ::"v"(fence0));
        } else {
#pragma unroll
            for (int k = 0; k < CS_ITERS; ++k) K1_COMMIT1(k, 0);
        }
    }
    __syncthreads();
    base_init(cs.head_pos(0) > 0);

    for (int kt = 0; kt < nt; ++kt) {
        const int half_a = kt & 1;
        auto unit = [&](auto par) __attribute__((always_inline)) {
            constexpr int PAR = decltype(par)::value;
            constexpr int cb = PAR;
            const unsigned char* const tile = cs_smem + cb * TILE_BYTES;
            h8 X[4][2], Wv[2][2];
#define CS_PX(g_, r_, part_) (*reinterpret_cast<const h8*>(tile + (paddr[(g_) >> 1] ^ (((part_) ? lo_xor : 0) | (((g_) & 1) << 5))) + (r_) * (CS_IW * 128)))
#define CS_WT(g_, ky_, part_) (*reinterpret_cast<const h8*>(wlane + (((g_) * 3 + (ky_)) << 12) + ((part_) << 10)))
            X[0][0] = CS_PX(0, 0, 0);
            X[0][1] = CS_PX(0, 0, 1);
            X[1][0] = CS_PX(0, 1, 0);
            X[1][1] = CS_PX(0, 1, 1);
            Wv[0][0] = CS_WT(0, 0, 0);
            Wv[0][1] = CS_WT(0, 0, 1);
            __builtin_amdgcn_sched_barrier(0);
            [[maybe_unused]] unsigned fence_w = 0;
            const __amdgpu_buffer_rsrc_t rsf = __builtin_amdgcn_make_buffer_rsrc(const_cast<float*>(p.bias), 0, 256, 0x00020000);
            if constexpr (PAR == 1) {
                K1_DMA_W(half_a ^ 1, 2);
                fence_w = __builtin_amdgcn_raw_buffer_load_b32(rsf, 0, 0, 0);
            }
            const int q_item = PAR == 0 ? c_item : n_item, y0q = PAR == 0 ? c_y0 : n_y0, x0q = PAR == 0 ? c_x0 : n_x0;
            const int q_half = half_a ^ 1;
            const __amdgpu_buffer_rsrc_t rs = __builtin_amdgcn_make_buffer_rsrc(
                const_cast<float*>(p.in) + (size_t)q_item * H * W * 64, 0, item_bytes, 0x00020000);
            const int org = ((y0q - 1) * W + x0q - 1) * 256 + q_half * 128;
            const bool interior = y0q > 0 && y0q + CS_IH - 1 <= H && x0q > 0 && x0q + CS_IW - 1 <= W;
            if constexpr (!ISF) K1_REQUEST_ALL(rs, org, interior, y0q, x0q);
            [[maybe_unused]] f32x16 bias16;
            if constexpr (PAR == 0) {
#pragma unroll
                for (int q = 0; q < 4; ++q) {
                    const f32x4 b4 = *reinterpret_cast<const f32x4*>(bl + ech + 4 * q);
                    bias16[4 * q] = b4.x;
                    bias16[4 * q + 1] = b4.y;
                    bias16[4 * q + 2] = b4.z;
                    bias16[4 * q + 3] = b4.w;
                }
            }
            [[maybe_unused]] u32x4 w10[8];
            auto substep = [&](auto sc) __attribute__((always_inline)) {
                constexpr int S = decltype(sc)::value;
                constexpr int g = S / 3, ky = S % 3;
                if constexpr (PAR == 1 && S == K1_W10_AT) {
                    const u32x4* src = reinterpret_cast<const u32x4*>(p.wpack2) + ((size_t)fch * 16 + 2 * mt) * 64 + lane;
#pragma unroll
                    for (int q = 0; q < 4; ++q) {
                        w10[2 * q] = src[(4 * q) * 64];
                        w10[2 * q + 1] = src[(4 * q + 1) * 64];
                    }
                }
                if constexpr (PAR == 0 && S >= 1 && S <= 8) held_store(S - 1, p.out);
                if constexpr (ky == 0) {
                    if constexpr (g == 2) {
                        if constexpr (PAR == 1) asm volatile("" ::"v"(fence_w));
                        K1_BARRIER();
                        if constexpr (PAR == 0) K1_DMA_W(half_a ^ 1, 0);
                        if constexpr (ISF) {
                            K1_DMA_HALO(rs, org, interior, y0q, x0q, cb ^ 1);
                            if constexpr (PAR == 1) fence_w = __builtin_amdgcn_raw_buffer_load_b32(rsf, 0, 0, 0);
                        }
                    }
                    if constexpr (g == 3 && PAR == 0) {
                        const int kn = min(kt + 1, nt - 1);
                        decode(kn, n_item, n_y0, n_x0, n_f);
                    }
                    if constexpr (g == 4) {
                        K1_BARRIER();
                        if constexpr (PAR == 0) {
                            K1_DMA_W(half_a ^ 1, 1);
                            fence_w = __builtin_amdgcn_raw_buffer_load_b32(rsf, 0, 0, 0);
                        }
                        if constexpr (!ISF) {
#pragma unroll
                            for (int k = 0; k < CS_ITERS; ++k) asm volatile("" : "+v"(lpk[k]));
#pragma unroll
                            for (int k = 0; k < CS_ITERS / 2; ++k) K1_COMMIT1(k, cb ^ 1);
                        }
                    }
                    if constexpr (g == 5 && !ISF) {
#pragma unroll
                        for (int k = CS_ITERS / 2; k < CS_ITERS; ++k) K1_COMMIT1(k, cb ^ 1);
                    }
                }
                __builtin_amdgcn_sched_barrier(0);
                {
                    constexpr int S1 = S + 1, g1 = S1 / 3, ky1 = S1 % 3;
                    constexpr bool RD = S < 17;
                    constexpr bool FIRST = PAR == 0 && S == 0;
                    const f32x16 zero = {0.f, 0.f, 0.f, 0.f, 0.f, 0.f, 0.f, 0.f, 0.f, 0.f, 0.f, 0.f, 0.f, 0.f, 0.f, 0.f};
                    const h8 wh = Wv[S & 1][0], wo = Wv[S & 1][1];
                    accm[0] = mfma_f16(wh, X[ky][0], FIRST ? bias16 : accm[0]);
                    __builtin_amdgcn_sched_barrier(0);
                    if constexpr (RD) {
                        Wv[S1 & 1][0] = CS_WT(g1, ky1, 0);
                        Wv[S1 & 1][1] = CS_WT(g1, ky1, 1);
                    }
                    __builtin_amdgcn_sched_barrier(0);
                    accm[1] = mfma_f16(wh, X[ky + 1][0], FIRST ? bias16 : accm[1]);
                    __builtin_amdgcn_sched_barrier(0);
                    if constexpr (RD) {
                        if constexpr (ky1 == 0) {
                            X[0][0] = CS_PX(g1, 0, 0);
                            X[0][1] = CS_PX(g1, 0, 1);
                        } else {
                            X[ky1 + 1][0] = CS_PX(g1, ky1 + 1, 0);
                            X[ky1 + 1][1] = CS_PX(g1, ky1 + 1, 1);
                        }
                    }
                    __builtin_amdgcn_sched_barrier(0);
                    accc[0] = mfma_f16(wo, X[ky][0], FIRST ? zero : accc[0]);
                    __builtin_amdgcn_sched_barrier(0);
                    if constexpr (RD && ky1 == 0) {
                        X[1][0] = CS_PX(g1, 1, 0);
                        X[1][1] = CS_PX(g1, 1, 1);
                    }
                    __builtin_amdgcn_sched_barrier(0);
                    accc[1] = mfma_f16(wo, X[ky + 1][0], FIRST ? zero : accc[1]);
                    accc[0] = mfma_f16(wh, X[ky][1], accc[0]);
                    accc[1] = mfma_f16(wh, X[ky + 1][1], accc[1]);
                }
                __builtin_amdgcn_sched_barrier(0);
            };
            substep(std::integral_constant<int, 0>{});
            substep(std::integral_constant<int, 1>{});
            substep(std::integral_constant<int, 2>{});
            substep(std::integral_constant<int, 3>{});
            substep(std::integral_constant<int, 4>{});
            substep(std::integral_constant<int, 5>{});
            substep(std::integral_constant<int, 6>{});
            substep(std::integral_constant<int, 7>{});
            substep(std::integral_constant<int, 8>{});
            substep(std::integral_constant<int, 9>{});
            substep(std::integral_constant<int, 10>{});
            substep(std::integral_constant<int, 11>{});
            substep(std::integral_constant<int, 12>{});
            substep(std::integral_constant<int, 13>{});
            substep(std::integral_constant<int, 14>{});
            substep(std::integral_constant<int, 15>{});
            substep(std::integral_constant<int, 16>{});
            substep(std::integral_constant<int, 17>{});
#undef CS_PX
#undef CS_WT
            if constexpr (PAR == 1) {
                RowHalves h0, h1;
#pragma unroll
                for (int q = 0; q < 4; ++q) quarter_prep(h0, accm[0], accc[0], q, true);
                if constexpr (ISF) asm volatile("" ::"v"(fence_w));
                K1_BARRIER();
                row_dump(h0);
                K1_BARRIER();
                row_pass(0, std::true_type{}, w10, &held[0], [&](int q) __attribute__((always_inline)) { quarter_prep(h1, accm[1], accc[1], q, true); });
                K1_BARRIER();
                row_dump(h1);
                K1_BARRIER();
                row_pass(1, std::true_type{}, w10, &held[4], [&](int) __attribute__((always_inline)) {});
                hx0 = c_x0;
                hy0 = c_y0;
                hitem = c_item;
                hpend = true;
                const bool is_part = cs.in_part(kt);
                const bool last = fch + 1 == cs.end_pos(kt, gT);
                if (last && is_part) {
#pragma unroll
                    for (int j = 0; j < 8; ++j) held_store(j, p.out);
                    float* const pt = p.partial + (size_t)cs.slot * (CS_TH * CS_TW * 64) + (size_t)(2 * rp * CS_TW + (lane & 31)) * 64 + ech;
#pragma unroll
                    for (int n = 0; n < 2; ++n)
#pragma unroll
                        for (int q = 0; q < 4; ++q)
                            *reinterpret_cast<f32x4*>(pt + n * (CS_TW * 64) + 4 * q) =
                                f32x4{base_m[n][4 * q], base_m[n][4 * q + 1], base_m[n][4 * q + 2], base_m[n][4 * q + 3]};
                    hpend = false;
                } else if (last) {
#pragma unroll
                    for (int j = 0; j < 8; ++j) held_store(j, p.out);
                    hitem = c_item / gT;
                    RowHalves hb0, hb1;
#pragma unroll
                    for (int q = 0; q < 4; ++q) {
                        quarter_prep(hb0, base_m[0], base_m[0], q, false);
                        quarter_prep(hb1, base_m[1], base_m[1], q, false);
                    }
                    K1_BARRIER();
                    row_dump(hb0);
                    K1_BARRIER();
                    row_pass(0, std::false_type{}, w10, &held[0], [&](int) __attribute__((always_inline)) {});
                    K1_BARRIER();
                    row_dump(hb1);
                    K1_BARRIER();
                    row_pass(1, std::false_type{}, w10, &held[4], [&](int) __attribute__((always_inline)) {});
#pragma unroll
                    for (int j = 0; j < 8; ++j) held_store(j, p.out2);
                    hpend = false;
                    base_init(cs.head_pos(kt + 1) > 0);
                }
                if constexpr (SPLIT) fch = n_f;
                else fch = last ? 0 : fch + 1;
                c_item = n_item;
                c_y0 = n_y0;
                c_x0 = n_x0;
            } else {
                asm volatile("" ::"v"(fence_w));
                K1_BARRIER();
            }
        };
        unit(std::integral_constant<int, 0>{});
        unit(std::integral_constant<int, 1>{});
    }
#pragma unroll
    for (int j = 0; j < 8; ++j) held_store(j, p.out);
#undef K1_DMA_HALO
#undef K1_REQUEST_ALL
#undef K1_COMMIT1
#undef K1_BARRIER
#undef K1_DMA_W
}

static bool split_params_ok(const ConvSplitParams& p, int grid) {
    return p.split_s == 0 || split_geometry_ok(p.H, p.W, p.items, p.add_div, p.n_full, p.split_s, p.split_q, grid);
}

__global__ __launch_bounds__(256) void c10_finalize_kernel(ConvSplitParams p) {
    const int H = p.H, W = p.W;
    const int tiles_x = (W + CS_TW - 1) / CS_TW, tiles_y = (H + CS_TH - 1) / CS_TH;
    const int per_item = tiles_x * tiles_y;
    const int j = blockIdx.x >> 3, ch = p.n_full + j;
    int clip, y0, x0;
    chain_tile(ch, per_item, tiles_x, 1, 0, clip, y0, x0);
    const float slope = p.act ? 0.2f : 1.0f;
    const int S = p.split_s;
#pragma unroll
    for (int it = 0; it < 2; ++it) {
        const int id = (blockIdx.x & 7) * 512 + it * 256 + threadIdx.x;
        const int pix = id >> 4, c4 = id & 15;
        const int y = y0 + pix / CS_TW, x = x0 + (pix & (CS_TW - 1));
        const float* src = p.partial + ((size_t)j * S * (CS_TH * CS_TW) + pix) * 64 + c4 * 4;
        f32x4 part[7];
#pragma unroll
        for (int r = 0; r < 7; ++r) part[r] = r < S ? *reinterpret_cast<const f32x4*>(src + (size_t)r * (CS_TH * CS_TW * 64)) : f32x4{0.f, 0.f, 0.f, 0.f};
        f32x4 v = part[0];
#pragma unroll
        for (int r = 1; r < 7; ++r)
            if (r < S) v += part[r];
        if (p.out) v += *reinterpret_cast<const f32x4*>(p.bias + c4 * 4);
        v.x = fmaxf(v.x, slope * v.x);
        v.y = fmaxf(v.y, slope * v.y);
        v.z = fmaxf(v.z, slope * v.z);
        v.w = fmaxf(v.w, slope * v.w);
        const h4 hi = __builtin_convertvector(v, h4);
        const h4 lo = __builtin_convertvector((v - __builtin_convertvector(hi, f32x4)) * CS_SCALE, h4);
        if (p.out) {
            if (y < H && x < W) *reinterpret_cast<f32x4*>(p.out + (((size_t)clip * H + y) * W + x) * 64 + c4 * 4) = v;
        } else if (y < H && x < W) {
            unsigned char* dst = reinterpret_cast<unsigned char*>(p.out2) + (((size_t)clip * H + y) * W + x) * 256 + (c4 >> 3) * 128 + (c4 & 7) * 8;
            *reinterpret_cast<h4*>(dst) = hi;
            *reinterpret_cast<h4*>(dst + 64) = lo;
        }
    }
}

hipError_t launch_c10_finalize(const ConvSplitParams& p, hipStream_t s) {
    if (!p.partial || (!p.out2 == !p.out) || (p.out && !p.bias) || p.items < 1 || p.H < 1 || p.W < 1 || p.add_div < 1 || p.items % p.add_div) return hipErrorInvalidValue;
    if (!split_geometry_ok(p.H, p.W, p.items, p.add_div, p.n_full, p.split_s, p.split_q, persistent_grid(device_cu_count()))) return hipErrorInvalidValue;
    const long long nchains = (long long)((p.W + CS_TW - 1) / CS_TW) * ((p.H + CS_TH - 1) / CS_TH) * (p.items / p.add_div);
    hipLaunchKernelGGL(c10_finalize_kernel, dim3((unsigned)(nchains - p.n_full) * 8), dim3(256), 0, s, p);
    return hipGetLastError();
}

hipError_t launch_conv3x3_c1c10(const ConvSplitParams& p, hipStream_t s) {
    if (!p.in || !p.wpack || !p.bias || !p.wpack2 || !p.bias2 || !p.out || !p.out2 || p.items < 1 || p.H < 1 || p.W < 1) return hipErrorInvalidValue;
    if (p.add_div < 1 || p.add_div > 7 || p.items % p.add_div || p.addend || p.resid || p.accum) return hipErrorInvalidValue;
    if ((long long)p.H * p.W * 256 >= 0x7fffffffLL) return hipErrorInvalidValue;
    int dev = 0;
    if (hipGetDevice(&dev) != hipSuccess || dev < 0 || dev >= 64) return hipErrorInvalidDevice;
    const int ncu = device_cu_count();
    if (!ncu) return hipErrorUnknown;
    const int grid = persistent_grid(ncu);
    if (!split_params_ok(p, grid) || (p.split_s && !p.partial)) return hipErrorInvalidValue;
    static std::atomic<int> attr_dev[64][4];
    const int isf = p.in_sf ? 1 : 0;
    const int var = isf + (p.split_s ? 2 : 0);
    const void* const fns[4] = {reinterpret_cast<const void*>(conv3x3_c1c10_kernel<false, false>), reinterpret_cast<const void*>(conv3x3_c1c10_kernel<true, false>),
                                reinterpret_cast<const void*>(conv3x3_c1c10_kernel<false, true>), reinterpret_cast<const void*>(conv3x3_c1c10_kernel<true, true>)};
    const int lds = isf ? K1_SF_LDS_BYTES : K1_LDS_BYTES;
    if (!attr_dev[dev][var]) {
        hipError_t e = hipFuncSetAttribute(fns[var], hipFuncAttributeMaxDynamicSharedMemorySize, lds);
        if (e != hipSuccess) return e;
        attr_dev[dev][var] = 1;
    }
    switch (var) {
        case 0: hipLaunchKernelGGL((conv3x3_c1c10_kernel<false, false>), dim3(grid), dim3(CS_THREADS), lds, s, p); break;
        case 1: hipLaunchKernelGGL((conv3x3_c1c10_kernel<true, false>), dim3(grid), dim3(CS_THREADS), lds, s, p); break;
        case 2: hipLaunchKernelGGL((conv3x3_c1c10_kernel<false, true>), dim3(grid), dim3(CS_THREADS), lds, s, p); break;
        default: hipLaunchKernelGGL((conv3x3_c1c10_kernel<true, true>), dim3(grid), dim3(CS_THREADS), lds, s, p); break;
    }
    return hipGetLastError();
}

hipError_t launch_conv3x3_split16(const ConvSplitParams& p, hipStream_t s) {
    if (!p.in || !p.wpack || !p.bias || !p.out || p.items < 1 || p.H < 1 || p.W < 1) return hipErrorInvalidValue;
    if ((p.addend == nullptr) != (p.resid == nullptr) || (p.addend && (p.add_div < 1 || p.items % p.add_div))) return hipErrorInvalidValue;
    if (p.accum && (p.addend || p.add_div < 1 || p.items % p.add_div)) return hipErrorInvalidValue;
    if ((long long)p.H * p.W * 256 >= 0x7fffffffLL) return hipErrorInvalidValue;
    const int ncu = device_cu_count();
    if (!ncu) return hipErrorUnknown;
    const int grid = persistent_grid(ncu);
    static std::atomic<int> attr_dev[64][4];
    int dev = 0;
    if (hipGetDevice(&dev) != hipSuccess || dev < 0 || dev >= 64) return hipErrorInvalidDevice;
    if (p.out_sf && (p.accum || p.addend)) return hipErrorInvalidValue;
    if (p.split_s) {
        if (!p.accum || !p.partial || !split_params_ok(p, grid)) return hipErrorInvalidValue;
        static std::atomic<int> attr_split[64];
        if (!attr_split[dev]) {
            hipError_t e = hipFuncSetAttribute(reinterpret_cast<const void*>(conv3x3_split16_kernel<2, false, true>), hipFuncAttributeMaxDynamicSharedMemorySize, CS_LDS_BYTES);
            if (e != hipSuccess) return e;
            attr_split[dev] = 1;
        }
        hipLaunchKernelGGL((conv3x3_split16_kernel<2, false, true>), dim3(grid), dim3(CS_THREADS), CS_LDS_BYTES, s, p);
        return hipGetLastError();
    }
    const int mode = p.out_sf ? 3 : p.accum ? 2 : p.addend ? 1 : 0;
    const void* fn = mode == 3 ? reinterpret_cast<const void*>(conv3x3_split16_kernel<0, true>)
                   : mode == 2 ? reinterpret_cast<const void*>(conv3x3_split16_kernel<2>)
                   : mode     ? reinterpret_cast<const void*>(conv3x3_split16_kernel<1>) : reinterpret_cast<const void*>(conv3x3_split16_kernel<0>);
    if (!attr_dev[dev][mode]) {
        hipError_t e = hipFuncSetAttribute(fn, hipFuncAttributeMaxDynamicSharedMemorySize, CS_LDS_BYTES);
        if (e != hipSuccess) return e;
        attr_dev[dev][mode] = 1;
    }
    if (mode == 3) hipLaunchKernelGGL((conv3x3_split16_kernel<0, true>), dim3(grid), dim3(CS_THREADS), CS_LDS_BYTES, s, p);
    else if (mode == 2) hipLaunchKernelGGL(conv3x3_split16_kernel<2>, dim3(grid), dim3(CS_THREADS), CS_LDS_BYTES, s, p);
    else if (mode) hipLaunchKernelGGL(conv3x3_split16_kernel<1>, dim3(grid), dim3(CS_THREADS), CS_LDS_BYTES, s, p);
    else hipLaunchKernelGGL(conv3x3_split16_kernel<0>, dim3(grid), dim3(CS_THREADS), CS_LDS_BYTES, s, p);
    return hipGetLastError();
}

static int split_row_channel(int i) { return 16 * ((i >> 2) & 1) + 4 * (i >> 3) + (i & 3); }

static uint16_t f16_bits(float f) {
    const _Float16 h = (_Float16)f;
    uint16_t u;
    std::memcpy(&u, &h, 2);
    return u;
}

size_t conv3x3_split16_pack_halfs() { return 2 * (size_t)CS_W_BYTES / 2; }

void conv3x3_split16_pack_weights(const float* hwio, int cin_total, int cin_begin, uint16_t* dst, int cout, bool identity_rows) {
    for (int half = 0; half < 2; ++half)
        for (int kx = 0; kx < 3; ++kx)
            for (int ks = 0; ks < 2; ++ks)
                for (int ky = 0; ky < 3; ++ky)
                    for (int m = 0; m < 2; ++m)
                        for (int lane = 0; lane < 64; ++lane)
                            for (int e = 0; e < 8; ++e) {
                                const int ci = cin_begin + 32 * half + 16 * ks + 8 * (lane >> 5) + e;
                                const int co = 32 * m + (identity_rows ? (lane & 31) : split_row_channel(lane & 31));
                                const float w = co < cout ? hwio[((size_t)(ky * 3 + kx) * cin_total + ci) * cout + co] : 0.f;
                                const _Float16 hi = (_Float16)w;
                                const float lo = (w - (float)hi) * CS_SCALE;
                                const size_t base = (size_t)half * (CS_W_BYTES / 2) + ((((size_t)(kx * 2 + ks) * 3 + ky) * 2 + m) * 2) * 512;
                                dst[base + lane * 8 + e] = f16_bits((float)hi);
                                dst[base + 512 + lane * 8 + e] = f16_bits(lo);
                            }
}

void conv3x3_split16_pack_weights16(const float* hwio, int cin_total, int cin_begin, uint16_t* dst) {
    for (int half = 0; half < 2; ++half)
        for (int kx = 0; kx < 3; ++kx)
            for (int ky = 0; ky < 3; ++ky)
                for (int c4 = 0; c4 < 4; ++c4)
                    for (int lane = 0; lane < 64; ++lane)
                        for (int e = 0; e < 8; ++e) {
                            const int ci = cin_begin + 32 * half + 8 * (lane >> 4) + e;
                            const int co = 16 * c4 + (lane & 15);
                            const float w = hwio[((size_t)(ky * 3 + kx) * cin_total + ci) * 64 + co];
                            const _Float16 hi = (_Float16)w;
                            const float lo = (w - (float)hi) * CS_SCALE;
                            const size_t base = (size_t)half * (CS_W_BYTES / 2) + ((((size_t)(kx * 3 + ky) * 4 + c4) * 2) * 512);
                            dst[base + lane * 8 + e] = f16_bits((float)hi);
                            dst[base + 512 + lane * 8 + e] = f16_bits(lo);
                        }
}

size_t conv1x1_c10_pack_halfs(int T) { return (size_t)T * 8192; }

void conv1x1_c10_pack_weights(const float* hwio, int T, uint16_t* dst) {
    for (int f = 0; f < T; ++f)
        for (int q = 0; q < 4; ++q)
            for (int g = 0; g < 2; ++g)
                for (int lane = 0; lane < 64; ++lane)
                    for (int e = 0; e < 8; ++e) {
                        const int ci = f * 64 + 32 * (q >> 1) + 16 * (lane >> 5) + 8 * (q & 1) + e;
                        const int co = 32 * g + split_row_channel(lane & 31);
                        const float w = hwio[(size_t)ci * 64 + co];
                        const _Float16 hi = (_Float16)w;
                        const float lo = (w - (float)hi) * CS_SCALE;
                        const size_t base = (((((size_t)f * 4 + q) * 2 + g) * 2) * 64 + lane) * 8 + e;
                        dst[base] = f16_bits((float)hi);
                        dst[base + 512] = f16_bits(lo);
                    }
}

}
```

### pfnl_amd/ops.py

```python
from __future__ import annotations

import ctypes as C
from typing import Optional

import numpy as np

from . import _capi


def _req(t, name):
    import torch
    if not (isinstance(t, torch.Tensor) and t.is_cuda and t.dtype == torch.float32 and t.is_contiguous()):
        raise TypeError(f"{name} must be a contiguous float32 tensor on the GPU")
    return C.c_void_p(t.data_ptr())


def _req16(t, name):
    import torch
    if not (isinstance(t, torch.Tensor) and t.is_cuda and t.dtype == torch.bfloat16 and t.is_contiguous()):
        raise TypeError(f"{name} must be a contiguous bfloat16 tensor on the GPU")
    return C.c_void_p(t.data_ptr())


def _host(a, name) -> Optional[np.ndarray]:
# ... 310 lines not shown
    out = torch.empty((B, H, W, 3 * T), dtype=torch.float32, device=x.device)
    _capi.check(lib.pfnl_op_nonlocal_block(_req(x, "x"), *[_hp(a) for a in arrs], *[_hp(a) for a in proj], int(nltype),
                                           int(sub_sample), _req(out, "out"), B, T, H, W, _stream(x)))
    return out


def conv0(x, kernel, bias=None):
    import torch
    lib = _capi.load_library()
    B, T, H, W, c = x.shape
    k, b = _host(kernel, "kernel"), _host(bias, "bias")
    if k.shape != (5, 5, 3, 64) or c != 3:
        raise ValueError("conv0: geometry mismatch")
    out = torch.empty((B * T, H, W, 64), dtype=torch.float32, device=x.device)
    _capi.check(lib.pfnl_op_conv0(_req(x, "x"), _hp(k), _hp(b), _req(out, "out"), B, T, H, W, _stream(x)))
    return out


def tail(merge, x, kernel, bias, scale: int):
    import torch
    lib = _capi.load_library()
    B, T, H, W, c = x.shape
    k, b = _host(kernel, "kernel"), _host(bias, "bias")
    if merge.shape != (B, H, W, 48) or k.shape != (3, 3, 12, 12 if scale == 4 else 3):
        raise ValueError("tail: geometry mismatch")
    out = torch.empty((B, 1, scale * H, scale * W, 3), dtype=torch.float32, device=x.device)
    _capi.check(lib.pfnl_op_tail(_req(merge, "merge"), _req(x, "x"), _hp(k), _hp(b), _req(out, "out"), B, T, H, W, scale, _stream(x)))
    return out


def gather_windows(frames, first: int, count: int, num_frames: int):
    import torch
    lib = _capi.load_library()
    F, H, W, c = frames.shape
    if c != 3:
        raise ValueError("gather_windows expects [F,H,W,3]")
    out = torch.empty((count, num_frames, H, W, 3), dtype=torch.float32, device=frames.device)
    _capi.check(lib.pfnl_op_gather_windows(_req(frames, "frames"), _req(out, "out"), F, first, count, num_frames, H, W, _stream(frames)))
    return out


def quantise_u8(sr):
    import torch
    lib = _capi.load_library()
    _req(sr, "sr")
    out = torch.empty(sr.shape, dtype=torch.uint8, device=sr.device)
    _capi.check(lib.pfnl_op_quantise_u8(C.c_void_p(sr.data_ptr()), C.c_void_p(out.data_ptr()), sr.numel(), _stream(sr)))
    return out


def conv2_chain_ex(x, kernel, bias, base, resid, add_div: int, act: bool = True, mfma: int = 32, split=(0, 0, 0), out=None):
    import torch
    lib = _capi.load_library()
    F, H, W, c = x.shape
    k, b = _host(kernel, "kernel"), _host(bias, "bias")
    if c != 64 or k.shape != (3, 3, 128, 64) or F % add_div:
        raise ValueError("conv2_chain_ex: geometry mismatch")
    if out is None:
        out = torch.empty((F, H, W, 64), dtype=torch.float32, device=x.device)
    n_full, s, q = (int(v) for v in split)
    _capi.check(lib.pfnl_op_conv2_chain_ex(_req(x, "x"), _hp(k), _hp(b), _req(base, "base"), int(add_div), _req(resid, "resid"),
                                           _req(out, "out"), F, H, W, 1 if act else 0, int(mfma), n_full, s, q, _stream(x)))
    return out


def conv1_conv10_split16_ex(x, k1, b1, k10, b10, frames_per_clip: int, split=(0, 0, 0), out1=None, base=None):
    import torch
    lib = _capi.load_library()
    F, H, W, c = x.shape
    T = int(frames_per_clip)
    k1h, k10h = _host(k1, "k1"), _host(k10, "k10")
    if c != 64 or F % T or k1h.size != 9 * 64 * 64 or k10h.size != 64 * T * 64:
        raise ValueError("conv1_conv10_split16_ex: geometry mismatch")
    if out1 is None:
        out1 = torch.empty((F, H, W, 64), dtype=torch.float32, device=x.device)
    if base is None:
        base = torch.empty((F // T, H, W, 64), dtype=torch.float32, device=x.device)
    n_full, s, q = (int(v) for v in split)
    _capi.check(lib.pfnl_op_conv1_conv10_split16_ex(_req(x, "x"), _hp(k1h), _hp(_host(b1, "b1")), _hp(k10h), _hp(_host(b10, "b10")),
                                                    _req(out1, "out1"), _req(base, "base"), F // T, T, H, W, n_full, s, q, _stream(x)))
    return out1, base


def conv3x3_accum_split16_ex(x, kernel, bias=None, act=True, frames_per_clip=1, split=(0, 0, 0), out=None):
    import torch
    lib = _capi.load_library()
    k, b = _host(kernel, "kernel"), _host(bias, "bias")
    F, H, W, c = x.shape
    T = int(frames_per_clip)
    if k.shape[:3] != (3, 3, 64 * T) or c != 64 or F % T or k.shape[3] > 64:
        raise ValueError("conv3x3_accum_split16_ex: geometry mismatch")
    if out is None:
        out = torch.empty((F // T, H, W, 64), dtype=torch.float32, device=x.device)
    n_full, s, q = (int(v) for v in split)
    _capi.check(lib.pfnl_op_conv3x3_accum_split16_ex(_req(x, "x"), _hp(k), _hp(b), _req(out, "out"), F // T, T, H, W, int(k.shape[3]),
                                                     1 if act else 0, n_full, s, q, _stream(x)))
    return out


def conv3x3_bf16_ex(x, kernel, bias, addend, add_div, resid, act=True, mfma: int = 32, split=(0, 0, 0), out=None):
    import torch
    lib = _capi.load_library()
    k, b = _host(kernel, "kernel"), _host(bias, "bias")
    F, H, W, c = x.shape
    if k.shape != (3, 3, 64, 64) or c != 64 or F % add_div:
        raise ValueError("conv3x3_bf16_ex: geometry mismatch")
    if out is None:
        out = torch.empty_like(x)
    n_full, s, q = (int(v) for v in split)
    _capi.check(lib.pfnl_op_conv3x3_bf16_ex(_req16(x, "x"), _hp(k), _hp(b), _req16(addend, "addend"), int(add_div), _req16(resid, "resid"),
                                            _req16(out, "out"), F, H, W, 1 if act else 0, int(mfma), n_full, s, q, _stream(x)))
    return out


def conv1_conv10_bf16_ex(x, k1, b1, k10, b10, frames_per_clip, mfma: int = 32, split=(0, 0, 0), out1=None, base=None):
    import torch
    lib = _capi.load_library()
    k1h, b1h, k10h, b10h = _host(k1, "k1"), _host(b1, "b1"), _host(k10, "k10"), _host(b10, "b10")
    F, H, W, c = x.shape
    T = int(frames_per_clip)
    if k1h.shape != (3, 3, 64, 64) or k10h.shape != (1, 1, 64 * T, 64) or c != 64 or F % T:
        raise ValueError("conv1_conv10_bf16_ex: geometry mismatch")
    if out1 is None:
        out1 = torch.empty_like(x)
    if base is None:
        base = torch.empty((F // T, H, W, 64), dtype=torch.bfloat16, device=x.device)
    n_full, s, q = (int(v) for v in split)
    _capi.check(lib.pfnl_op_conv1_conv10_bf16_ex(_req16(x, "x"), _hp(k1h), _hp(b1h), _hp(k10h), _hp(b10h), _req16(out1, "out1"),
                                                 _req16(base, "base"), F // T, T, H, W, int(mfma), n_full, s, q, _stream(x)))
    return out1, base
```

Baseline: 915.9.

## Add 16x16x32 MFMA variant of fused conv1+conv10 kernel

After: 940.4 (median of 6 runs). 2.7% higher.

```diff
diff --git a/include/pfnl_hip.h b/include/pfnl_hip.h
--- a/include/pfnl_hip.h
+++ b/include/pfnl_hip.h
@@ -114,6 +114,9 @@
 int pfnl_op_conv1_conv10_split16_ex(const float* in, const float* k1_host, const float* b1_host, const float* k10_host,
                                     const float* b10_host, float* out1, float* base, int clips, int frames_per_clip, int H, int W,
                                     int n_full, int split_s, int split_q, void* stream);
+int pfnl_op_conv1_conv10_split16_mfma(const float* in, const float* k1_host, const float* b1_host, const float* k10_host,
+                                      const float* b10_host, float* out1, float* base, int clips, int frames_per_clip, int H, int W,
+                                      int mfma, int n_full, int split_s, int split_q, void* stream);
 int pfnl_op_conv3x3_accum_split16_ex(const float* in, const float* kernel_host, const float* bias_host, float* out, int clips,
                                      int frames_per_clip, int H, int W, int cout, int act, int n_full, int split_s, int split_q, void* stream);
 int pfnl_op_conv3x3_bf16_ex(const uint16_t* in, const float* kernel_host, const float* bias_host, const uint16_t* addend, int add_div,
diff --git a/pfnl_amd/_capi.py b/pfnl_amd/_capi.py
--- a/pfnl_amd/_capi.py
+++ b/pfnl_amd/_capi.py
@@ -77,6 +77,7 @@
     "pfnl_op_conv2_chain_sf0": (_i, [_vp, _vp, _vp, _vp, _i, _vp, _vp, _vp, _i, _i, _i, _i, _vp]),
     "pfnl_op_conv2_chain_ex": (_i, [_vp, _vp, _vp, _vp, _i, _vp, _vp, _i, _i, _i, _i, _i, _i, _i, _i, _vp]),
     "pfnl_op_conv1_conv10_split16_ex": (_i, [_vp, _vp, _vp, _vp, _vp, _vp, _vp, _i, _i, _i, _i, _i, _i, _i, _vp]),
+    "pfnl_op_conv1_conv10_split16_mfma": (_i, [_vp, _vp, _vp, _vp, _vp, _vp, _vp, _i, _i, _i, _i, _i, _i, _i, _i, _vp]),
     "pfnl_op_conv3x3_accum_split16_ex": (_i, [_vp, _vp, _vp, _vp, _i, _i, _i, _i, _i, _i, _i, _i, _i, _vp]),
     "pfnl_op_conv3x3_bf16_ex": (_i, [_vp, _vp, _vp, _vp, _i, _vp, _vp, _i, _i, _i, _i, _i, _i, _i, _i, _vp]),
     "pfnl_op_conv1_conv10_bf16_ex": (_i, [_vp, _vp, _vp, _vp, _vp, _vp, _vp, _i, _i, _i, _i, _i, _i, _i, _i, _vp]),
diff --git a/pfnl_amd/csrc/capi.hip b/pfnl_amd/csrc/capi.hip
--- a/pfnl_amd/csrc/capi.hip
+++ b/pfnl_amd/csrc/capi.hip
@@ -157,7 +157,7 @@
     size_t c1_w = 0, c1_b = 0, c10_w = 0, c10_b = 0, c10_s = 0, c2a_w = 0, c2b_w = 0, c2_b = 0;
     size_t c1_u = 0, c2a_u = 0, c2b_u = 0;
     size_t bf_c1 = 0, bf_c10 = 0, bf_c2a = 0, bf_c2b = 0, bf_c1_m16 = 0, bf_c2b_m16 = 0;
-    size_t s_c1 = 0, s_c2a = 0, s_c2b = 0, s_c10 = 0, s_c10f = 0, s_c2a_sf = 0, s_c2b_sf = 0, s_c2a_m16 = 0, s_c2b_m16 = 0;
+    size_t s_c1 = 0, s_c2a = 0, s_c2b = 0, s_c10 = 0, s_c10f = 0, s_c2a_sf = 0, s_c2b_sf = 0, s_c2a_m16 = 0, s_c2b_m16 = 0, s_c1_m16 = 0;
     size_t sm_c1 = 0, sm_c10 = 0, sm_c2 = 0;
 };
 
@@ -392,6 +392,7 @@
     int launches_per_block = 0;
     int tiles8x32 = 0, chains = 0;
     int mfma = 32;
+    int c1_mfma = 32;
     int merge1 = M1_DIRECT;
     int merge_stride = 48;
     size_t p10_floats = 0, inp0sf_floats = 0, c10part_floats = 0;
@@ -443,6 +444,7 @@
         pl.c1x1_launches = 1;
     }
     pl.mfma = (h->s16_m16 && pl.c10_fused && pl.chain && !pl.sf0 && !pl.split_s && pl.chains >= grid) ? 16 : 32;
+    pl.c1_mfma = pl.mfma;
     pl.name = pl.mid ? "mid4" : (pl.c10_fused && pl.chain) ? (pl.sf0 ? "chain2_sf0" : (pl.split_s ? "chain2_split" : "chain2"))
             : pl.algo == 4 ? (pl.launches_per_block == 3 ? "split16_3" : "split16_4")
             : pl.algo == 3 ? (pl.conv2_grouped ? "winograd_ws3" : "winograd_ws4")
@@ -686,6 +688,7 @@
             q.bias2 = wd + k.c10_b;
             q.out2 = h->base.p;
             set_split_chains(q, pl, h->c10part.p);
+            if (pl.c1_mfma == 16) q.wpack_m16 = f.w16s + k.s_c1_m16;
             HIPCHK(launch_conv3x3_c1c10(q, s));
         }
         if (pl.split_s) {
@@ -1244,7 +1247,7 @@
     {
         std::vector<uint16_t> b16;
         const size_t n3 = pfnl::conv3x3_split16_pack_halfs(), n1 = pfnl::conv1x1_split16_pack_halfs(T);
-        const size_t blk = 7 * n3 + n1 + pfnl::conv1x1_c10_pack_halfs(T);
+        const size_t blk = 8 * n3 + n1 + pfnl::conv1x1_c10_pack_halfs(T);
         h->off16s_m1 = (size_t)nb * blk;
         const size_t m3 = pfnl::conv_small_pack_halfs(3, 1), m10 = pfnl::conv_small_pack_halfs(1, T);
         const size_t small_base = (size_t)nb * blk + (size_t)T * n3;
@@ -1265,6 +1268,8 @@
             k.s_c10f = k.s_c2b_sf + n3;
             k.s_c2a_m16 = k.s_c10f + pfnl::conv1x1_c10_pack_halfs(T);
             k.s_c2b_m16 = k.s_c2a_m16 + n3;
+            k.s_c1_m16 = k.s_c2b_m16 + n3;
+            pfnl::conv3x3_split16_pack_weights16(W("conv1_" + s).data(), 64, 0, &b16[k.s_c1_m16], true);
             pfnl::conv3x3_split16_pack_weights16(W("conv2_" + s).data(), 128, 0, &b16[k.s_c2a_m16]);
             pfnl::conv3x3_split16_pack_weights16(W("conv2_" + s).data(), 128, 64, &b16[k.s_c2b_m16]);
             pfnl::conv1x1_c10_pack_weights(W("conv10_" + s).data(), T, &b16[k.s_c10f]);
@@ -1333,11 +1338,11 @@
                       nln[pl.nl_family], pl.nl_fused_pack ? 1 : 0, pl.mfma, kMerge1Names[pl.merge1]);
     else
         std::snprintf(tmp, sizeof tmp, "%s launches_per_block=%d c1x1=%d precision=fp32 conv3x3=%s conv1x1=%s c10_fused=%d chain=%d sf0=%d strict=%d tiles=%d chains=%d "
-                      "whole_chains=%d split_parts=%d part_frames=%d nl=%s nl_pack_fused=%d mfma=%d merge1=%s",
+                      "whole_chains=%d split_parts=%d part_frames=%d nl=%s nl_pack_fused=%d mfma=%d c1_mfma=%d merge1=%s",
                       pl.name, pl.launches_per_block, pl.c1x1_launches, pl.small ? "small" : a3[pl.algo < 0 || pl.algo > 4 ? 2 : pl.algo],
                       a1[pl.conv1x1_algo < 0 || pl.conv1x1_algo > 2 ? 0 : pl.conv1x1_algo], pl.c10_fused ? 1 : 0, pl.chain ? 1 : 0, pl.sf0 ? 1 : 0,
                       pl.strict ? 1 : 0, pl.tiles8x32, pl.chains, pl.split_s ? pl.n_full : pl.chains, pl.split_s, pl.split_q, nln[pl.nl_family],
-                      pl.nl_fused_pack ? 1 : 0, pl.mfma, kMerge1Names[pl.merge1]);
+                      pl.nl_fused_pack ? 1 : 0, pl.mfma, pl.c1_mfma, kMerge1Names[pl.merge1]);
     if (std::strlen(tmp) + 1 > buflen) return fail(PFNL_ERR_INVALID, "buffer too small");
     std::strcpy(buf, tmp);
     return 0;
diff --git a/pfnl_amd/csrc/capi_ops.hip b/pfnl_amd/csrc/capi_ops.hip
--- a/pfnl_amd/csrc/capi_ops.hip
+++ b/pfnl_amd/csrc/capi_ops.hip
@@ -152,14 +152,15 @@
 
 static int op_conv1_conv10_split16(const float* in, const float* k1_host, const float* b1_host, const float* k10_host,
                                    const float* b10_host, float* out1, float* base, int clips, int frames_per_clip, int H, int W,
-                                   void* stream, bool in_sf, int n_full = 0, int split_s = 0, int split_q = 0) {
+                                   void* stream, bool in_sf, int n_full = 0, int split_s = 0, int split_q = 0, bool m16 = false) {
     if (!in || !k1_host || !k10_host || !out1 || !base) return fail(PFNL_ERR_INVALID, "NULL argument");
     const int T = frames_per_clip;
     if (clips < 1 || T < 1 || T > 7 || H < 1 || W < 1) return fail(PFNL_ERR_INVALID, "unsupported conv geometry");
     OpStage st(stream);
     const size_t n3 = pfnl::conv3x3_split16_pack_halfs(), n1 = pfnl::conv1x1_c10_pack_halfs(T);
-    std::vector<uint16_t> pack(n3 + n1 + 256, 0);
+    std::vector<uint16_t> pack(n3 + n1 + 256 + (m16 ? n3 : 0), 0);
     pfnl::conv3x3_split16_pack_weights(k1_host, 64, 0, pack.data());
+    if (m16) pfnl::conv3x3_split16_pack_weights16(k1_host, 64, 0, pack.data() + n3 + n1 + 256, true);
     pfnl::conv1x1_c10_pack_weights(k10_host, T, pack.data() + n3);
     if (b1_host) std::memcpy(&pack[n3 + n1], b1_host, 64 * sizeof(float));
     if (b10_host) std::memcpy(&pack[n3 + n1 + 128], b10_host, 64 * sizeof(float));
@@ -180,6 +181,7 @@
         q.split_s = split_s;
         q.split_q = split_q;
         q.partial = part;
+        if (m16) q.wpack_m16 = dw + n3 + n1 + 256;
         return pfnl::launch_conv3x3_c1c10(q, st.s);
     });
     if (split_s) st.run([&] {
@@ -668,6 +670,20 @@
     return op_conv1_conv10_split16(in, k1_host, b1_host, k10_host, b10_host, out1, base, clips, T, H, W, stream, false, n_full, split_s, split_q);
 }
 
+int pfnl_op_conv1_conv10_split16_mfma(const float* in, const float* k1_host, const float* b1_host, const float* k10_host,
+                                      const float* b10_host, float* out1, float* base, int clips, int frames_per_clip, int H, int W,
+                                      int mfma, int n_full, int split_s, int split_q, void* stream) {
+    if (mfma != 16 && mfma != 32) return fail(PFNL_ERR_INVALID, "mfma must be 16 or 32");
+    if (mfma == 16 && split_s) return fail(PFNL_ERR_INVALID, "split chains run on the 32x32x16 kernel only");
+    if (mfma == 32) return pfnl_op_conv1_conv10_split16_ex(in, k1_host, b1_host, k10_host, b10_host, out1, base, clips, frames_per_clip, H, W, n_full, split_s, split_q, stream);
+    if (!in || !k1_host || !k10_host || !out1 || !base) return fail(PFNL_ERR_INVALID, "NULL argument");
+    const int T = frames_per_clip;
+    if (clips < 1 || T < 1 || T > 7 || H < 1 || W < 1) return fail(PFNL_ERR_INVALID, "unsupported conv geometry");
+    if (int r = frame_too_large(H, W, 256)) return r;
+    if (!split_args_ok(H, W, clips * T, T, n_full, split_s, split_q)) return fail(PFNL_ERR_INVALID, "invalid split-chain geometry");
+    return op_conv1_conv10_split16(in, k1_host, b1_host, k10_host, b10_host, out1, base, clips, T, H, W, stream, false, n_full, 0, split_q, true);
+}
+
 int pfnl_op_conv3x3_accum_split16_ex(const float* in, const float* kernel_host, const float* bias_host, float* out, int clips,
                                      int frames_per_clip, int H, int W, int cout, int act, int n_full, int split_s, int split_q, void* stream) {
     if (!in || !kernel_host || !out) return fail(PFNL_ERR_INVALID, "NULL argument");
diff --git a/pfnl_amd/csrc/conv_split16.h b/pfnl_amd/csrc/conv_split16.h
--- a/pfnl_amd/csrc/conv_split16.h
+++ b/pfnl_amd/csrc/conv_split16.h
@@ -31,7 +31,8 @@
 
 hipError_t launch_conv3x3_split16(const ConvSplitParams& p, hipStream_t s);
 size_t conv3x3_split16_pack_halfs();
-void conv3x3_split16_pack_weights16(const float* hwio, int cin_total, int cin_begin, uint16_t* dst);
+void conv3x3_split16_pack_weights16(const float* hwio, int cin_total, int cin_begin, uint16_t* dst,
+                                    bool perm_rows = false);
 void conv3x3_split16_pack_weights(const float* hwio, int cin_total, int cin_begin, uint16_t* dst, int cout = 64,
                                   bool identity_rows = false);
 
diff --git a/pfnl_amd/csrc/conv_split16.hip b/pfnl_amd/csrc/conv_split16.hip
--- a/pfnl_amd/csrc/conv_split16.hip
+++ b/pfnl_amd/csrc/conv_split16.hip
@@ -535,8 +535,14 @@
 constexpr int K1_SF_LDS_BYTES = 2 * K1_SF_TILE_BYTES + CS_W_BYTES + 2 * 64 * 4;
 static_assert(K1_SF_LDS_BYTES <= 160 * 1024, "LDS budget");
 
-template <bool ISF, bool SPLIT>
+#define K1_SWZ16(px_) ((((px_) >> 1) & 3) << 1)
+typedef float k1f4 __attribute__((ext_vector_type(4)));
+__device__ __forceinline__ k1f4 k1_mfma16(h8 a, h8 b, k1f4 c) {
+    return __builtin_amdgcn_mfma_f32_16x16x32_f16(a, b, c, 0, 0, 0);
+}
+template <bool ISF, bool SPLIT, bool M16 = false>
 __global__ __launch_bounds__(CS_THREADS, 1) void conv3x3_c1c10_kernel(ConvSplitParams p) {
+    static_assert(!M16 || (!ISF && !SPLIT), "16x16x32 form: whole rounds, fp32 input");
     constexpr int TILE_BYTES = ISF ? K1_SF_TILE_BYTES : CS_TILE_BYTES;
     extern __shared__ __attribute__((aligned(16))) unsigned char cs_smem[];
     unsigned char* const wl = cs_smem + 2 * TILE_BYTES;
@@ -600,16 +606,17 @@
         const int id = k * CS_THREADS + tid < CS_PIECES ? k * CS_THREADS + tid : CS_PIECES - 8 + (tid & 7);
         int pix = id >> 3;
         const int c = id & 7;
-        if (pix < (CS_IH * CS_IW & ~15)) pix = (pix & ~15) | ((pix & 1) << 3) | ((pix & 15) >> 1);
+        if (pix < (CS_IH * CS_IW & ~15)) pix = M16 ? ((pix & ~7) | ((pix & 1) << 2) | ((pix & 7) >> 1)) : ((pix & ~15) | ((pix & 1) << 3) | ((pix & 15) >> 1));
         const int py = pix / CS_IW, px = pix - py * CS_IW;
-        lpk[k] = ((py * CS_IW + px) * 128 + 8 * (c & 1) + (((c >> 1) ^ ((px >> 1) & 7)) << 4)) | (py << 16) | (px << 24);
+        lpk[k] = ((py * CS_IW + px) * 128 + 8 * (c & 1) + (((c >> 1) ^ (M16 ? K1_SWZ16(px) : ((px >> 1) & 7))) << 4)) | (py << 16) | (px << 24);
     }
     const int c16 = (tid & 7) * 16;
     const float nscale = __builtin_bit_cast(float, __builtin_amdgcn_readfirstlane(__builtin_bit_cast(int, -CS_SCALE)));
     [[maybe_unused]] f32x4 stg[CS_ITERS];
-#define K1_REQUEST_ALL(rs_, org_, interior_, y0_, x0_)                                           \
+#define K1_REQUEST_ALL(rs_, org_, interior_, y0_, x0_) K1_REQUEST(0, CS_ITERS, rs_, org_, interior_, y0_, x0_)
+#define K1_REQUEST(k0_, k1_, rs_, org_, interior_, y0_, x0_)                                     \
     do {                                                                                         \
-        _Pragma("unroll") for (int k_ = 0; k_ < CS_ITERS; ++k_) {                                \
+        _Pragma("unroll") for (int k_ = (k0_); k_ < (k1_); ++k_) {                               \
             const int py_ = (lpk[k_] >> 16) & 0xff, px_ = (unsigned)lpk[k_] >> 24;               \
             const int gy_ = (y0_) + py_ - 1, gx_ = (x0_) + px_ - 1;                              \
             const bool in_ = (interior_) | (((unsigned)gy_ < (unsigned)H) & ((unsigned)gx_ < (unsigned)W));    \
@@ -630,14 +637,25 @@
     int paddr[3];
 #pragma unroll
     for (int kx = 0; kx < 3; ++kx) {
-        const int col = (lane & 31) + kx;
-        paddr[kx] = ((2 * rp) * CS_IW + col) * 128 + ((((lane >> 5)) ^ ((col >> 1) & 7)) << 4);
+        const int col = (lane & (M16 ? 15 : 31)) + kx;
+        paddr[kx] = M16 ? ((2 * rp) * CS_IW + col) * 128 + (((lane >> 4) ^ K1_SWZ16(col)) << 4)
+                        : ((2 * rp) * CS_IW + col) * 128 + ((((lane >> 5)) ^ ((col >> 1) & 7)) << 4);
     }
     const int lo_xor = 4 << 4;
-    const unsigned char* const wlane = wl + mt * 2048 + lane * 16;
+    const unsigned char* const wlane = wl + mt * (M16 ? 4096 : 2048) + lane * 16;
     const int kh = lane >> 5;
     const int ech = 32 * mt + 16 * kh;
     f32x16 accm[2], accc[2], base_m[2];
+    [[maybe_unused]] k1f4 am16[2][4], ac16[2][4];
+    if constexpr (M16) {
+#pragma unroll
+        for (int n = 0; n < 2; ++n)
+#pragma unroll
+            for (int q = 0; q < 4; ++q) {
+                am16[n][q] = k1f4{0.f, 0.f, 0.f, 0.f};
+                ac16[n][q] = k1f4{0.f, 0.f, 0.f, 0.f};
+            }
+    }
     u32x4 held[8];
     int hx0 = 0, hy0 = 0, hitem = 0;
     bool hpend = false;
@@ -673,6 +691,15 @@
         asm("v_max_f32 %0, %1, %2" : "=v"(t.w) : "v"(t.w), "v"(st.w));
         split4(t, h.hi[q], h.lo[q], nscale);
     };
+    [[maybe_unused]] auto quarter_prep4 = [&](RowHalves& h, const k1f4& m, const k1f4& c, int q) __attribute__((always_inline)) {
+        f32x4 t = f32x4{m[0], m[1], m[2], m[3]} + f32x4{c[0], c[1], c[2], c[3]} * CS_ISCALE;
+        const f32x4 st = mul4s(t, slope);
+        asm("v_max_f32 %0, %1, %2" : "=v"(t.x) : "v"(t.x), "v"(st.x));
+        asm("v_max_f32 %0, %1, %2" : "=v"(t.y) : "v"(t.y), "v"(st.y));
+        asm("v_max_f32 %0, %1, %2" : "=v"(t.z) : "v"(t.z), "v"(st.z));
+        asm("v_max_f32 %0, %1, %2" : "=v"(t.w) : "v"(t.w), "v"(st.w));
+        split4(t, h.hi[q], h.lo[q], nscale);
+    };
     const int pp = rp * 32 + (lane & 31);
     const int sw = pp & 15;
     unsigned char* const pl = scratch + pp * 256;
@@ -682,6 +709,15 @@
         *reinterpret_cast<u32x4*>(pl + (((c0 + 1) ^ sw) << 4)) = u32x4{h.hi[2].x, h.hi[2].y, h.hi[3].x, h.hi[3].y};
         *reinterpret_cast<u32x4*>(pl + (((c0 + 4) ^ sw) << 4)) = u32x4{h.lo[0].x, h.lo[0].y, h.lo[1].x, h.lo[1].y};
         *reinterpret_cast<u32x4*>(pl + (((c0 + 5) ^ sw) << 4)) = u32x4{h.lo[2].x, h.lo[2].y, h.lo[3].x, h.lo[3].y};
+    };
+    [[maybe_unused]] auto row_dump16 = [&](const RowHalves& h) __attribute__((always_inline)) {
+        const int n16 = lane & 15, c0 = 8 * mt + (lane >> 4);
+#pragma unroll
+        for (int ph = 0; ph < 2; ++ph) {
+            unsigned char* const plx = scratch + (rp * 32 + 16 * ph + n16) * 256;
+            *reinterpret_cast<u32x4*>(plx + ((c0 ^ n16) << 4)) = u32x4{h.hi[2 * ph].x, h.hi[2 * ph].y, h.hi[2 * ph + 1].x, h.hi[2 * ph + 1].y};
+            *reinterpret_cast<u32x4*>(plx + (((c0 + 4) ^ n16) << 4)) = u32x4{h.lo[2 * ph].x, h.lo[2 * ph].y, h.lo[2 * ph + 1].x, h.lo[2 * ph + 1].y};
+        }
     };
     auto row_pass = [&](int n, auto mm, const u32x4 (&w10)[8], u32x4* pc, auto&& fill) __attribute__((always_inline)) {
         constexpr bool MM = decltype(mm)::value;
@@ -769,12 +805,31 @@
             h8 X[4][2], Wv[2][2];
 #define CS_PX(g_, r_, part_) (*reinterpret_cast<const h8*>(tile + (paddr[(g_) >> 1] ^ (((part_) ? lo_xor : 0) | (((g_) & 1) << 5))) + (r_) * (CS_IW * 128)))
 #define CS_WT(g_, ky_, part_) (*reinterpret_cast<const h8*>(wlane + (((g_) * 3 + (ky_)) << 12) + ((part_) << 10)))
-            X[0][0] = CS_PX(0, 0, 0);
-            X[0][1] = CS_PX(0, 0, 1);
-            X[1][0] = CS_PX(0, 1, 0);
-            X[1][1] = CS_PX(0, 1, 1);
-            Wv[0][0] = CS_WT(0, 0, 0);
-            Wv[0][1] = CS_WT(0, 0, 1);
+            if constexpr (!M16) {
+                X[0][0] = CS_PX(0, 0, 0);
+                X[0][1] = CS_PX(0, 0, 1);
+                X[1][0] = CS_PX(0, 1, 0);
+                X[1][1] = CS_PX(0, 1, 1);
+                Wv[0][0] = CS_WT(0, 0, 0);
+                Wv[0][1] = CS_WT(0, 0, 1);
+            }
+            [[maybe_unused]] h8 X6[4][2][2], W6[3][2][2];
+#define K1_PX16(kx_, ph_, r_, part_) (*reinterpret_cast<const h8*>(tile + (paddr[kx_] ^ ((part_) ? lo_xor : 0)) + (r_) * (CS_IW * 128) + (ph_) * 2048))
+#define K1_WT16(kx_, ky_, t_, part_) (*reinterpret_cast<const h8*>(wlane + (((kx_) * 3 + (ky_)) << 13) + (((t_) * 2 + (part_)) << 10)))
+            if constexpr (M16) {
+                W6[0][0][0] = K1_WT16(0, 0, 0, 0);
+                X6[0][0][0] = K1_PX16(0, 0, 0, 0);
+                W6[0][1][0] = K1_WT16(0, 0, 1, 0);
+                W6[0][0][1] = K1_WT16(0, 0, 0, 1);
+                X6[0][0][1] = K1_PX16(0, 0, 0, 1);
+                W6[0][1][1] = K1_WT16(0, 0, 1, 1);
+                X6[0][1][0] = K1_PX16(0, 1, 0, 0);
+                X6[0][1][1] = K1_PX16(0, 1, 0, 1);
+                X6[1][0][0] = K1_PX16(0, 0, 1, 0);
+                X6[1][1][0] = K1_PX16(0, 1, 1, 0);
+                X6[1][0][1] = K1_PX16(0, 0, 1, 1);
+                X6[1][1][1] = K1_PX16(0, 1, 1, 1);
+            }
             __builtin_amdgcn_sched_barrier(0);
             [[maybe_unused]] unsigned fence_w = 0;
             const __amdgpu_buffer_rsrc_t rsf = __builtin_amdgcn_make_buffer_rsrc(const_cast<float*>(p.bias), 0, 256, 0x00020000);
@@ -788,9 +843,15 @@
                 const_cast<float*>(p.in) + (size_t)q_item * H * W * 64, 0, item_bytes, 0x00020000);
             const int org = ((y0q - 1) * W + x0q - 1) * 256 + q_half * 128;
             const bool interior = y0q > 0 && y0q + CS_IH - 1 <= H && x0q > 0 && x0q + CS_IW - 1 <= W;
-            if constexpr (!ISF) K1_REQUEST_ALL(rs, org, interior, y0q, x0q);
+            if constexpr (!ISF && !M16) K1_REQUEST_ALL(rs, org, interior, y0q, x0q);
+            if constexpr (M16 && PAR == 1) K1_REQUEST(0, CS_ITERS / 2, rs, org, interior, y0q, x0q);
             [[maybe_unused]] f32x16 bias16;
-            if constexpr (PAR == 0) {
+            [[maybe_unused]] k1f4 bias4[2];
+            if constexpr (M16 && PAR == 0) {
+                bias4[0] = *reinterpret_cast<const k1f4*>(bl + 32 * mt + 8 * (lane >> 4));
+                bias4[1] = *reinterpret_cast<const k1f4*>(bl + 32 * mt + 8 * (lane >> 4) + 4);
+            }
+            if constexpr (PAR == 0 && !M16) {
 #pragma unroll
                 for (int q = 0; q < 4; ++q) {
                     const f32x4 b4 = *reinterpret_cast<const f32x4*>(bl + ech + 4 * q);
@@ -884,37 +945,133 @@
                 }
                 __builtin_amdgcn_sched_barrier(0);
             };
-            substep(std::integral_constant<int, 0>{});
-            substep(std::integral_constant<int, 1>{});
-            substep(std::integral_constant<int, 2>{});
-            substep(std::integral_constant<int, 3>{});
-            substep(std::integral_constant<int, 4>{});
-            substep(std::integral_constant<int, 5>{});
-            substep(std::integral_constant<int, 6>{});
-            substep(std::integral_constant<int, 7>{});
-            substep(std::integral_constant<int, 8>{});
-            substep(std::integral_constant<int, 9>{});
-            substep(std::integral_constant<int, 10>{});
-            substep(std::integral_constant<int, 11>{});
-            substep(std::integral_constant<int, 12>{});
-            substep(std::integral_constant<int, 13>{});
-            substep(std::integral_constant<int, 14>{});
-            substep(std::integral_constant<int, 15>{});
-            substep(std::integral_constant<int, 16>{});
-            substep(std::integral_constant<int, 17>{});
+            auto substep16 = [&](auto sc) __attribute__((always_inline)) {
+                constexpr int S = decltype(sc)::value;
+                constexpr int ky = S % 3;
+                if constexpr (PAR == 1 && S == 8) {
+                    const u32x4* src = reinterpret_cast<const u32x4*>(p.wpack2) + ((size_t)fch * 16 + 2 * mt) * 64 + lane;
+#pragma unroll
+                    for (int q = 0; q < 4; ++q) {
+                        w10[2 * q] = src[(4 * q) * 64];
+                        w10[2 * q + 1] = src[(4 * q + 1) * 64];
+                    }
+                }
+                if constexpr (PAR == 0 && S <= 3) {
+                    held_store(2 * S, p.out);
+                    held_store(2 * S + 1, p.out);
+                }
+                if constexpr (PAR == 0 && S == 1) K1_REQUEST(0, CS_ITERS / 2, rs, org, interior, y0q, x0q);
+                if constexpr (S == 3) {
+                    if constexpr (PAR == 1) asm volatile("" ::"v"(fence_w));
+                    K1_BARRIER();
+                    if constexpr (PAR == 0) K1_DMA_W(half_a ^ 1, 0);
+                }
+                if constexpr (S == 4) {
+                    if constexpr (PAR == 0) {
+                        const int kn = min(kt + 1, nt - 1);
+                        decode(kn, n_item, n_y0, n_x0, n_f);
+                    }
+#pragma unroll
+                    for (int k = 0; k < CS_ITERS / 2; ++k) asm volatile("" : "+v"(lpk[k]));
+#pragma unroll
+                    for (int k = 0; k < CS_ITERS / 2; ++k) K1_COMMIT1(k, cb ^ 1);
+                    K1_REQUEST(CS_ITERS / 2, CS_ITERS, rs, org, interior, y0q, x0q);
+                }
+                if constexpr (S == 6) {
+                    K1_BARRIER();
+                    if constexpr (PAR == 0) {
+                        K1_DMA_W(half_a ^ 1, 1);
+                        fence_w = __builtin_amdgcn_raw_buffer_load_b32(rsf, 0, 0, 0);
+                    }
+                }
+                if constexpr (S == 7) {
+#pragma unroll
+                    for (int k = CS_ITERS / 2; k < CS_ITERS; ++k) asm volatile("" : "+v"(lpk[k]));
+#pragma unroll
+                    for (int k = CS_ITERS / 2; k < CS_ITERS; ++k) K1_COMMIT1(k, cb ^ 1);
+                }
+                __builtin_amdgcn_sched_barrier(0);
+                constexpr bool FIRST = PAR == 0 && S == 0;
+                constexpr bool NX = S < 8;
+                constexpr int kx1 = (S + 1) / 3, ky1 = (S + 1) % 3;
+                const k1f4 zero4 = k1f4{0.f, 0.f, 0.f, 0.f};
+#define K1_MM(n_, t_, ph_) do { am16[n_][2 * (ph_) + (t_)] = k1_mfma16(W6[ky][t_][0], X6[ky + (n_)][ph_][0], FIRST ? bias4[t_] : am16[n_][2 * (ph_) + (t_)]); __builtin_amdgcn_sched_barrier(0); } while (0)
+#define K1_CA(n_, t_, ph_) do { ac16[n_][2 * (ph_) + (t_)] = k1_mfma16(W6[ky][t_][1], X6[ky + (n_)][ph_][0], FIRST ? zero4 : ac16[n_][2 * (ph_) + (t_)]); __builtin_amdgcn_sched_barrier(0); } while (0)
+#define K1_CB(n_, t_, ph_) do { ac16[n_][2 * (ph_) + (t_)] = k1_mfma16(W6[ky][t_][0], X6[ky + (n_)][ph_][1], ac16[n_][2 * (ph_) + (t_)]); __builtin_amdgcn_sched_barrier(0); } while (0)
+#define K1_LW(t_, part_) do { if constexpr (NX) W6[ky1][t_][part_] = K1_WT16(kx1, ky1, t_, part_); __builtin_amdgcn_sched_barrier(0); } while (0)
+#define K1_LX(r_, ph_, part_) do { if constexpr (NX) X6[r_][ph_][part_] = K1_PX16(kx1, ph_, r_, part_); __builtin_amdgcn_sched_barrier(0); } while (0)
+                K1_MM(0, 0, 0); K1_MM(0, 1, 0); K1_CA(0, 0, 0); K1_CB(0, 0, 0); K1_CA(0, 1, 0); K1_CB(0, 1, 0);
+                K1_MM(0, 0, 1); K1_LW(0, 0);
+                K1_MM(0, 1, 1); K1_LW(0, 1);
+                K1_CA(0, 0, 1); K1_CB(0, 0, 1); K1_CA(0, 1, 1); K1_CB(0, 1, 1);
+                K1_MM(1, 0, 0); K1_LW(1, 0);
+                K1_MM(1, 0, 1); K1_CA(1, 0, 0); K1_LW(1, 1);
+                K1_CB(1, 0, 0); K1_CA(1, 0, 1); K1_CB(1, 0, 1);
+                K1_MM(1, 1, 0); K1_LX(ky1 != 0 ? ky + 2 : 0, 0, 0);
+                K1_MM(1, 1, 1); K1_CA(1, 1, 0); K1_LX(ky1 != 0 ? ky + 2 : 0, 0, 1);
+                K1_CB(1, 1, 0); K1_CA(1, 1, 1); K1_CB(1, 1, 1);
+                K1_LX(ky1 != 0 ? ky + 2 : 0, 1, 0); K1_LX(ky1 != 0 ? ky + 2 : 0, 1, 1);
+                if constexpr (ky1 == 0) { K1_LX(1, 0, 0); K1_LX(1, 0, 1); K1_LX(1, 1, 0); K1_LX(1, 1, 1); }
+#undef K1_MM
+#undef K1_CA
+#undef K1_CB
+#undef K1_LW
+#undef K1_LX
+                __builtin_amdgcn_sched_barrier(0);
+            };
+            if constexpr (M16) {
+                substep16(std::integral_constant<int, 0>{});
+                substep16(std::integral_constant<int, 1>{});
+                substep16(std::integral_constant<int, 2>{});
+                substep16(std::integral_constant<int, 3>{});
+                substep16(std::integral_constant<int, 4>{});
+                substep16(std::integral_constant<int, 5>{});
+                substep16(std::integral_constant<int, 6>{});
+                substep16(std::integral_constant<int, 7>{});
+                substep16(std::integral_constant<int, 8>{});
+            } else {
+                substep(std::integral_constant<int, 0>{});
+                substep(std::integral_constant<int, 1>{});
+                substep(std::integral_constant<int, 2>{});
+                substep(std::integral_constant<int, 3>{});
+                substep(std::integral_constant<int, 4>{});
+                substep(std::integral_constant<int, 5>{});
+                substep(std::integral_constant<int, 6>{});
+                substep(std::integral_constant<int, 7>{});
+                substep(std::integral_constant<int, 8>{});
+                substep(std::integral_constant<int, 9>{});
+                substep(std::integral_constant<int, 10>{});
+                substep(std::integral_constant<int, 11>{});
+                substep(std::integral_constant<int, 12>{});
+                substep(std::integral_constant<int, 13>{});
+                substep(std::integral_constant<int, 14>{});
+                substep(std::integral_constant<int, 15>{});
+                substep(std::integral_constant<int, 16>{});
+                substep(std::integral_constant<int, 17>{});
+            }
+#undef K1_PX16
+#undef K1_WT16
 #undef CS_PX
 #undef CS_WT
             if constexpr (PAR == 1) {
                 RowHalves h0, h1;
 #pragma unroll
-                for (int q = 0; q < 4; ++q) quarter_prep(h0, accm[0], accc[0], q, true);
+                for (int q = 0; q < 4; ++q) {
+                    if constexpr (M16) quarter_prep4(h0, am16[0][q], ac16[0][q], q);
+                    else quarter_prep(h0, accm[0], accc[0], q, true);
+                }
                 if constexpr (ISF) asm volatile("" ::"v"(fence_w));
                 K1_BARRIER();
-                row_dump(h0);
+                if constexpr (M16) row_dump16(h0);
+                else row_dump(h0);
                 K1_BARRIER();
-                row_pass(0, std::true_type{}, w10, &held[0], [&](int q) __attribute__((always_inline)) { quarter_prep(h1, accm[1], accc[1], q, true); });
+                row_pass(0, std::true_type{}, w10, &held[0], [&](int q) __attribute__((always_inline)) {
+                    if constexpr (M16) quarter_prep4(h1, am16[1][q], ac16[1][q], q);
+                    else quarter_prep(h1, accm[1], accc[1], q, true);
+                });
                 K1_BARRIER();
-                row_dump(h1);
+                if constexpr (M16) row_dump16(h1);
+                else row_dump(h1);
                 K1_BARRIER();
                 row_pass(1, std::true_type{}, w10, &held[4], [&](int) __attribute__((always_inline)) {});
                 hx0 = c_x0;
@@ -974,6 +1131,7 @@
     for (int j = 0; j < 8; ++j) held_store(j, p.out);
 #undef K1_DMA_HALO
 #undef K1_REQUEST_ALL
+#undef K1_REQUEST
 #undef K1_COMMIT1
 #undef K1_BARRIER
 #undef K1_DMA_W
@@ -1040,11 +1198,13 @@
     if (!ncu) return hipErrorUnknown;
     const int grid = persistent_grid(ncu);
     if (!split_params_ok(p, grid) || (p.split_s && !p.partial)) return hipErrorInvalidValue;
-    static std::atomic<int> attr_dev[64][4];
+    static std::atomic<int> attr_dev[64][5];
     const int isf = p.in_sf ? 1 : 0;
-    const int var = isf + (p.split_s ? 2 : 0);
-    const void* const fns[4] = {reinterpret_cast<const void*>(conv3x3_c1c10_kernel<false, false>), reinterpret_cast<const void*>(conv3x3_c1c10_kernel<true, false>),
-                                reinterpret_cast<const void*>(conv3x3_c1c10_kernel<false, true>), reinterpret_cast<const void*>(conv3x3_c1c10_kernel<true, true>)};
+    const bool m16 = p.wpack_m16 && !p.split_s && !isf;
+    const int var = m16 ? 4 : isf + (p.split_s ? 2 : 0);
+    const void* const fns[5] = {reinterpret_cast<const void*>(conv3x3_c1c10_kernel<false, false>), reinterpret_cast<const void*>(conv3x3_c1c10_kernel<true, false>),
+                                reinterpret_cast<const void*>(conv3x3_c1c10_kernel<false, true>), reinterpret_cast<const void*>(conv3x3_c1c10_kernel<true, true>),
+                                reinterpret_cast<const void*>(conv3x3_c1c10_kernel<false, false, true>)};
     const int lds = isf ? K1_SF_LDS_BYTES : K1_LDS_BYTES;
     if (!attr_dev[dev][var]) {
         hipError_t e = hipFuncSetAttribute(fns[var], hipFuncAttributeMaxDynamicSharedMemorySize, lds);
@@ -1055,6 +1215,12 @@
         case 0: hipLaunchKernelGGL((conv3x3_c1c10_kernel<false, false>), dim3(grid), dim3(CS_THREADS), lds, s, p); break;
         case 1: hipLaunchKernelGGL((conv3x3_c1c10_kernel<true, false>), dim3(grid), dim3(CS_THREADS), lds, s, p); break;
         case 2: hipLaunchKernelGGL((conv3x3_c1c10_kernel<false, true>), dim3(grid), dim3(CS_THREADS), lds, s, p); break;
+        case 4: {
+            ConvSplitParams q = p;
+            q.wpack = p.wpack_m16;
+            hipLaunchKernelGGL((conv3x3_c1c10_kernel<false, false, true>), dim3(grid), dim3(CS_THREADS), lds, s, q);
+            break;
+        }
         default: hipLaunchKernelGGL((conv3x3_c1c10_kernel<true, true>), dim3(grid), dim3(CS_THREADS), lds, s, p); break;
     }
     return hipGetLastError();
@@ -1129,7 +1295,7 @@
                             }
 }
 
-void conv3x3_split16_pack_weights16(const float* hwio, int cin_total, int cin_begin, uint16_t* dst) {
+void conv3x3_split16_pack_weights16(const float* hwio, int cin_total, int cin_begin, uint16_t* dst, bool perm_rows) {
     for (int half = 0; half < 2; ++half)
         for (int kx = 0; kx < 3; ++kx)
             for (int ky = 0; ky < 3; ++ky)
@@ -1137,7 +1303,8 @@
                     for (int lane = 0; lane < 64; ++lane)
                         for (int e = 0; e < 8; ++e) {
                             const int ci = cin_begin + 32 * half + 8 * (lane >> 4) + e;
-                            const int co = 16 * c4 + (lane & 15);
+                            const int r = lane & 15;
+                            const int co = perm_rows ? 32 * (c4 >> 1) + 8 * (r >> 2) + 4 * (c4 & 1) + (r & 3) : 16 * c4 + r;
                             const float w = hwio[((size_t)(ky * 3 + kx) * cin_total + ci) * 64 + co];
                             const _Float16 hi = (_Float16)w;
                             const float lo = (w - (float)hi) * CS_SCALE;
diff --git a/pfnl_amd/ops.py b/pfnl_amd/ops.py
--- a/pfnl_amd/ops.py
+++ b/pfnl_amd/ops.py
@@ -416,6 +416,25 @@
     return out1, base
 
 
+def conv1_conv10_split16_mfma(x, k1, b1, k10, b10, frames_per_clip: int, mfma: int = 16, split=(0, 0, 0), out1=None, base=None):
+    import torch
+    lib = _capi.load_library()
+    F, H, W, c = x.shape
+    T = int(frames_per_clip)
+    k1h, k10h = _host(k1, "k1"), _host(k10, "k10")
+    if c != 64 or F % T or k1h.size != 9 * 64 * 64 or k10h.size != 64 * T * 64:
+        raise ValueError("conv1_conv10_split16_mfma: geometry mismatch")
+    if out1 is None:
+        out1 = torch.empty((F, H, W, 64), dtype=torch.float32, device=x.device)
+    if base is None:
+        base = torch.empty((F // T, H, W, 64), dtype=torch.float32, device=x.device)
+    n_full, s, q = (int(v) for v in split)
+    _capi.check(lib.pfnl_op_conv1_conv10_split16_mfma(_req(x, "x"), _hp(k1h), _hp(_host(b1, "b1")), _hp(k10h), _hp(_host(b10, "b10")),
+                                                      _req(out1, "out1"), _req(base, "base"), F // T, T, H, W, int(mfma), n_full, s, q,
+                                                      _stream(x)))
+    return out1, base
+
+
 def conv3x3_accum_split16_ex(x, kernel, bias=None, act=True, frames_per_clip=1, split=(0, 0, 0), out=None):
     import torch
     lib = _capi.load_library()
```
